# LemonATsu/UNet-PhaseGen

Measured on NVIDIA B200. Metric: audio_seconds_per_second_mag_to_phase_to_wave, higher is better.
Workload: dtype f16x3/f16x2/f16-fp32acc (two-product fp16 on d1,u2; single fp16 product = TF32 operand rounding on u1)

## Files before the change

unet-phasegen_b200/csrc/api.cu:

```cuda
#include <cstdarg>
#include <cstdio>

#include "common.cuh"
#include "conv_plan.h"

namespace pg {
static thread_local char g_err[512] = "";

void set_error(const char* fmt, ...) {
    va_list ap;
    va_start(ap, fmt);
    vsnprintf(g_err, sizeof(g_err), fmt, ap);
    va_end(ap);
}

int check_launch(const char* what) {
    cudaError_t e = cudaGetLastError();
    if (e != cudaSuccess) {
        set_error("%s: launch failed: %s", what, cudaGetErrorString(e));
        return PG_ERR_CUDA;
    }
    return PG_OK;
}
}

extern "C" const char* pg_last_error(void) { return pg::g_err; }
extern "C" int pg_abi_version(void) { return 4; }

extern "C" int pg_check_device(int* sm_count, int* cc_major, int* cc_minor) {
    int dev = 0, n = 0;
    if (cudaGetDeviceCount(&n) != cudaSuccess || n == 0) {
        cudaGetLastError();
        pg::set_error("no CUDA device: the phasegen path has no CPU fallback");
        return PG_ERR_CUDA;
    }
    cudaGetDevice(&dev);
    cudaDeviceProp p;
    if (cudaGetDeviceProperties(&p, dev) != cudaSuccess) { pg::set_error("cudaGetDeviceProperties failed"); return PG_ERR_CUDA; }
    if (sm_count) *sm_count = p.multiProcessorCount;
    if (cc_major) *cc_major = p.major;
    if (cc_minor) *cc_minor = p.minor;
    if (p.major != 10) {
        pg::set_error("device '%s' is sm_%d%d; this library is built for sm_100a (B200) only", p.name, p.major, p.minor);
        return PG_ERR_UNSUPPORTED;
    }
    return PG_OK;
}

extern "C" int pg_conv_stat_parts(const pg_conv_desc* d) {
    if (!d) return PG_ERR_INVALID;
    pg::ConvPlan pl;
    int rc = pg::conv_plan_build(d, &pl);
    if (rc != PG_OK) return rc;
    return pl.OS * pl.n_ntiles;
}

extern "C" int pg_conv_tc_plan(const pg_conv_desc* d, int* out, int n_out) {
    PG_REQUIRE(d && out && n_out >= 16, "pg_conv_tc_plan: need a descriptor and room for 16 ints");
    pg::ConvPlan p;
    int rc = pg::conv_plan_build(d, &p);
    if (rc != PG_OK) return rc;
    const int v[16] = {p.n_tile, p.n_ntiles, p.nb, p.strip_rows, p.pair, p.merged, p.mgroups, p.acc_stages,
                       p.n_chunks, p.n_cotiles, p.OS, p.IS, p.n_taps[0], p.n_taps[1], p.n_groups[0], p.n_groups[1]};
    for (int i = 0; i < 16; ++i) out[i] = v[i];
    if (n_out >= 17) out[16] = p.whole_clip;
    return PG_OK;
}
```

unet-phasegen_b200/csrc/conv_plan.h:

```cpp
#pragma once
#include <stdint.h>
#include <stdlib.h>

#include "../../include/phasegen.h"
#include "common.cuh"

namespace pg {

constexpr int kMaxTaps = 32;

struct ConvTap { int8_t w_idx; int8_t shift; int8_t parity; int8_t pad_; int32_t d; };
struct ConvGroup { int32_t row0; int8_t parity; int8_t n_taps; int8_t first_tap; int8_t pad_; };

struct ConvPlan {
    int B, C_in, C_out, L_in, L_out, k;
    int IS, OS;
    int n_tile, n_ntiles;
    int n_chunks, n_cotiles;
    int strip_rows;
    int nb;
    int acc_stages;
    int pair;
    int mgroups;
    int merged;
    int clip_group;
    int whole_clip;
    int out_rows, out_ld;
    int n_groups[2], n_taps[2];
    ConvGroup groups[2][kMaxTaps];
    ConvTap taps[2][kMaxTaps];
};

static inline int floordiv(int a, int b) { return (a >= 0) ? a / b : -((-a + b - 1) / b); }

static inline int conv_plan_build(const pg_conv_desc* d, ConvPlan* p) {
    const int s = d->stride, k = d->k, pad = d->pad;
    if (s < 1 || s > 2 || k < 1 || k > kMaxTaps) { set_error("conv plan: stride must be 1 or 2 and k <= %d (got s=%d k=%d)", kMaxTaps, s, k); return PG_ERR_UNSUPPORTED; }
    const bool tr = d->kind == PG_CONV_TRANSPOSE;
    const int L_expect = tr ? (d->L_in - 1) * s - 2 * pad + k : (d->L_in + 2 * pad - k) / s + 1;
    const bool len_ok = tr ? (d->L_out >= L_expect && d->L_out < L_expect + s) : d->L_out == L_expect;
    if (!len_ok || d->L_out < 1) { set_error("conv plan: L_out %d does not match geometry (expected %d)", d->L_out, L_expect); return PG_ERR_INVALID; }
    p->B = d->B; p->C_in = d->C_in; p->C_out = d->C_out; p->L_in = d->L_in; p->L_out = d->L_out; p->k = k;
    p->IS = tr ? 1 : s;
    p->OS = tr ? s : 1;
    p->out_rows = d->out_rows; p->out_ld = d->out_ld;
    p->n_chunks = d->C_in / 64; p->n_cotiles = d->C_out / 128;
    const int l_max = (d->L_out + p->OS - 1) / p->OS;
    p->n_ntiles = (l_max + 255) / 256;
    p->n_tile = (((l_max + p->n_ntiles - 1) / p->n_ntiles) + 15) / 16 * 16;
    int tpg = d->taps_per_group <= 0 ? 16 : d->taps_per_group;
    int max_shift = 0;
    for (int phi = 0; phi < 2; ++phi) { p->n_groups[phi] = 0; p->n_taps[phi] = 0; }
    for (int phi = 0; phi < p->OS; ++phi) {
        ConvTap t[kMaxTaps]; int n = 0;
        for (int kk = 0; kk < k; ++kk) {
            ConvTap e; e.w_idx = (int8_t)kk; e.shift = 0; e.pad_ = 0;
            if (tr) {
                int num = phi + pad - kk;
                if (((num % s) + s) % s != 0) continue;
                e.parity = 0; e.d = floordiv(num, s);
            } else {
                int off = kk - pad;
                int q = ((off % s) + s) % s;
                e.parity = (int8_t)q; e.d = (off - q) / s;
            }
            t[n++] = e;
        }
        for (int i = 1; i < n; ++i) {
            ConvTap e = t[i]; int j = i - 1;
            while (j >= 0 && (t[j].parity > e.parity || (t[j].parity == e.parity && t[j].d > e.d))) { t[j + 1] = t[j]; --j; }
            t[j + 1] = e;
        }
        int ng = 0, i = 0;
        while (i < n) {
            ConvGroup g; g.parity = t[i].parity; g.row0 = t[i].d; g.first_tap = (int8_t)i; g.pad_ = 0;
            int j = i;
            while (j < n && t[j].parity == g.parity && (j - i) < tpg && (t[j].d - g.row0) < tpg &&
                   (p->n_tile + (t[j].d - g.row0) <= 256)) {
                t[j].shift = (int8_t)(t[j].d - g.row0);
                if (t[j].shift > max_shift) max_shift = t[j].shift;
                ++j;
            }
            g.n_taps = (int8_t)(j - i);
            p->groups[phi][ng++] = g;
            i = j;
        }
        for (int q = 0; q < n; ++q) p->taps[phi][q] = t[q];
        p->n_groups[phi] = ng; p->n_taps[phi] = n;
    }
    p->pair = (d->tc_cta_pair != 1 && d->C_out % 256 == 0 && d->precision != PG_PREC_FP32_SIMT) ? 1 : 0;
    if (d->tc_cta_pair == 2 && !p->pair) { set_error("conv plan: CTA pairs need C_out %% 256 == 0 (got %d)", d->C_out); return PG_ERR_INVALID; }
    const int n_cta = p->pair ? p->n_tile / 2 : p->n_tile;
    p->strip_rows = (n_cta + max_shift + 7) / 8 * 8;
    if (p->strip_rows > 256) p->strip_rows = 256;
    p->nb = 1;
    const bool weight_bound = d->precision == PG_PREC_F16X2 || d->precision == PG_PREC_BF16 || d->precision == PG_PREC_F16;
    if ((p->n_ntiles == 1 || weight_bound) && d->max_clips_per_tile != 1) {
        const int planes = (d->precision == PG_PREC_BF16X3 || d->precision == PG_PREC_F16X3 || d->precision == PG_PREC_F16X2) ? 2 : 1;
        const int max_rows = (72 * 1024) / (planes * 128);
        int nb = 512 / p->n_tile;
        if (nb * p->strip_rows > max_rows) nb = max_rows / p->strip_rows;
        if (nb * p->n_tile <= 256 || (p->n_tile > 128 && !weight_bound)) {
            nb = 256 / p->n_tile;
            if (nb * p->strip_rows > 256) nb = 256 / p->strip_rows;
        }
        if (nb > 16) nb = 16;
        if (d->max_clips_per_tile > 1 && nb > d->max_clips_per_tile) nb = d->max_clips_per_tile;
        if (nb > d->B) nb = d->B;
        if (nb < 1) nb = 1;
        p->nb = nb;
    }
    if (const char* e = getenv("PG_TC_NB")) {
        int nb = atoi(e);
        if (nb >= 1 && nb * p->n_tile <= 512 && nb <= d->B) p->nb = nb;
    }
    p->merged = 0; p->mgroups = 1;
    {
        const int strip_full = (p->n_tile + max_shift + 7) / 8 * 8;
        const int step = p->pair ? 2 : 1;
        int nb_max = 256 / strip_full;
        if (nb_max > d->B) nb_max = d->B;
        if (d->max_clips_per_tile > 1 && nb_max > d->max_clips_per_tile) nb_max = d->max_clips_per_tile;
        nb_max -= nb_max % step;
        const char* off = getenv("PG_TC_MERGED");
        if (p->n_ntiles == 1 && nb_max >= 2 && d->max_clips_per_tile != 1 && !(off && atoi(off) == 0)) {
            const int units = (d->tc_max_ctas > 0 ? d->tc_max_ctas : 148) / (p->pair ? 2 : 1);
            const int slabs = (p->pair ? p->n_cotiles / 2 : p->n_cotiles) * p->OS;
            long best = -1; int best_nb = step;
            for (int nb = step; nb <= nb_max; nb += step) {
                const long tiles = (long)slabs * ((d->B + nb - 1) / nb);
                const long cost = ((tiles + units - 1) / units) * (64 + (long)nb * strip_full);
                if (best < 0 || cost <= best) { best = cost; best_nb = nb; }
            }
            p->merged = 1; p->nb = best_nb; p->strip_rows = strip_full;
            const char* g2 = getenv("PG_TC_MGROUPS");
            const int g_cap = g2 ? atoi(g2) : 2;
            const int planes_b = (d->precision == PG_PREC_BF16X3 || d->precision == PG_PREC_F16X3 || d->precision == PG_PREC_F16X2) ? 2 : 1;
            const char* fr = getenv("PG_TC_MG_FRAC");
            const double need = (fr ? atof(fr) : 0.8) * units;
            for (int g = 4; g >= 2 && weight_bound; --g) {
                if (g > g_cap || g * best_nb > d->B || g * best_nb * strip_full > 512) continue;
                const long tiles_g = (long)slabs * ((d->B + g * best_nb - 1) / (g * best_nb));
                const long slot_bytes = (long)planes_b * (g * best_nb / (p->pair ? 2 : 1)) * strip_full * 128;
                if ((double)tiles_g < need || 2 * slot_bytes > 120 * 1024) continue;
                p->mgroups = g; p->nb = g * best_nb;
                break;
            }
        }
    }
    p->whole_clip = 0;
    if (d->tc_whole_clip) {
        const int parts = p->OS * p->n_ntiles;
        if (p->merged && p->OS > 1) {
            set_error("conv plan: merged two-phase tiles do not hold a whole clip");
            return PG_ERR_UNSUPPORTED;
        }
        if (!p->merged) {
            if (parts * p->n_tile > 512) { set_error("conv plan: a whole clip needs %d accumulator columns (> 512)", parts * p->n_tile); return PG_ERR_UNSUPPORTED; }
            if (parts > 1) {
                p->whole_clip = 1;
                int nb = 1;
                if (weight_bound && 2 * parts * p->n_tile <= 512) nb = 2;
                if (nb > d->B) nb = d->B;
                const int planes = (d->precision == PG_PREC_BF16X3 || d->precision == PG_PREC_F16X3 || d->precision == PG_PREC_F16X2) ? 2 : 1;
                if (nb * p->n_ntiles * p->strip_rows * planes * 128 > 72 * 1024) nb = 1;
                if (p->n_ntiles * p->strip_rows * planes * 128 > 80 * 1024) {
                    set_error("conv plan: the %d strips of a whole clip (%d rows each) do not fit shared memory", p->n_ntiles, p->strip_rows);
                    return PG_ERR_UNSUPPORTED;
                }
                p->nb = nb;
            }
        }
    }
    {
        const int cols = p->merged ? p->nb * p->strip_rows : p->nb * p->n_tile * (p->whole_clip ? p->OS * p->n_ntiles : 1);
        if (cols > 512) { set_error("conv plan: tile needs %d accumulator columns (> 512)", cols); return PG_ERR_UNSUPPORTED; }
        p->acc_stages = cols <= 256 ? 2 : 1;
    }
    p->clip_group = d->B;
    return PG_OK;
}

}
```

unet-phasegen_b200/csrc/conv_tc.cu:

```cuda
#include "tc_ptx.cuh"
#include "conv_plan.h"

namespace pg {

struct ConvTcParams {
    ConvPlan plan;
    float* y;
    float4* stats;
    int n_a_slots;
    int b_slot_bytes;
    int n_terms;
    int f16;
    int base_offset_mode;
    int a_mn;
    int epi_mode;
    const float* gamma; const float* beta; float eps;
    ActDst dst0, dst1;
    float2* ss_out;
    const int* clip_rows;
};

constexpr int kThreads = 192;
constexpr int kATileBytes = 128 * 128;
constexpr int kMaxASlots = 8;

struct TileCoord { int co_tile, phase, b0, nt; };

__device__ __forceinline__ int n_bundles(const ConvPlan& p) { return (p.B + p.nb - 1) / p.nb; }
__device__ __forceinline__ int n_co_slabs(const ConvPlan& p) { return p.pair ? p.n_cotiles / 2 : p.n_cotiles; }
__device__ __forceinline__ int tile_OS(const ConvPlan& p) { return p.whole_clip ? 1 : p.OS; }
__device__ __forceinline__ int tile_NT(const ConvPlan& p) { return p.whole_clip ? 1 : p.n_ntiles; }
__device__ __forceinline__ int total_tiles(const ConvPlan& p) { return n_co_slabs(p) * tile_OS(p) * n_bundles(p) * tile_NT(p); }
__device__ __forceinline__ TileCoord decode_tile(const ConvPlan& p, int tile) {
    TileCoord c;
    const int OSx = tile_OS(p), NTx = tile_NT(p);
    const int nbg = n_bundles(p), G = p.clip_group, n_slabs = n_co_slabs(p) * OSx;
    const int tiles_full = n_slabs * G * NTx;
    const int g = tile / tiles_full, r = tile % tiles_full;
    int Gg = nbg - g * G; if (Gg > G) Gg = G;
    const int per_slab = Gg * NTx;
    const int slab = r / per_slab, r2 = r % per_slab;
    c.co_tile = slab / OSx; c.phase = slab % OSx;
    c.b0 = (g * G + r2 / NTx) * p.nb; c.nt = r2 % NTx;
    return c;
}

template <bool PAIR, bool RAGGED>
__global__ void __launch_bounds__(kThreads, 1)
conv_tc_kernel(const __grid_constant__ CUtensorMap map_w_hi, const __grid_constant__ CUtensorMap map_w_lo,
               const __grid_constant__ CUtensorMap map_x_hi, const __grid_constant__ CUtensorMap map_x_lo,
               const __grid_constant__ ConvTcParams prm) {
    extern __shared__ __align__(1024) uint8_t smem_raw[];
    const ConvPlan& pl = prm.plan;
    uint8_t* smem = reinterpret_cast<uint8_t*>((reinterpret_cast<uintptr_t>(smem_raw) + 1023) & ~uintptr_t(1023));
    const int nA = prm.n_a_slots;
    const int bPlane = prm.b_slot_bytes;
    const int a_planes = prm.n_terms == 3 ? 2 : 1;
    const int b_planes = prm.n_terms >= 2 ? 2 : 1;
    uint8_t* a_base = smem;
    uint8_t* b_base = a_base + (size_t)nA * a_planes * kATileBytes;
    uint64_t* bars = reinterpret_cast<uint64_t*>(b_base + 2 * (size_t)b_planes * bPlane);
    uint64_t* fullA = bars;
    uint64_t* emptyA = bars + kMaxASlots;
    uint64_t* fullB = bars + 2 * kMaxASlots;
    uint64_t* emptyB = fullB + 2;
    uint64_t* accFull = emptyB + 2;
    uint64_t* accEmpty = accFull + 2;
    uint32_t* tmem_slot = reinterpret_cast<uint32_t*>(accEmpty + 2);
    uint32_t* epi_tiles = reinterpret_cast<uint32_t*>(reinterpret_cast<uint8_t*>(bars) + 256);

    const int warp = __shfl_sync(0xffffffffu, (int)(threadIdx.x >> 5), 0), lane = threadIdx.x & 31;
    const int n_tiles = total_tiles(pl);
    const bool w_lo = prm.n_terms == 3, x_lo = prm.n_terms >= 2;

    if (warp == 0 && lane == 0) {
        tma_prefetch_desc(&map_w_hi); tma_prefetch_desc(&map_x_hi);
        if (w_lo) tma_prefetch_desc(&map_w_lo);
        if (x_lo) tma_prefetch_desc(&map_x_lo);
        for (int i = 0; i < nA; ++i) { mbar_init(fullA + i, 1); mbar_init(emptyA + i, 1); }
        for (int i = 0; i < 2; ++i) {
            mbar_init(fullB + i, 1); mbar_init(emptyB + i, 1);
            mbar_init(accFull + i, 1); mbar_init(accEmpty + i, PAIR ? 8 : 4);
        }
        fence_barrier_init();
    }
    if (warp == 1) { if (PAIR) tmem_alloc_pair(tmem_slot, 512); else tmem_alloc(tmem_slot, 512); }
    tc_fence_before();
    if (PAIR) cluster_sync_all(); else __syncthreads();
    tc_fence_after();
    const uint32_t tmem_base = __shfl_sync(0xffffffffu, *tmem_slot, 0);
    const int rank = PAIR ? (int)cluster_ctarank() : 0;
    const int tile0 = PAIR ? (int)(blockIdx.x >> 1) : (int)blockIdx.x;
    const int tile_step = PAIR ? (int)(gridDim.x >> 1) : (int)gridDim.x;
    const int half_n = pl.n_tile >> 1;
    const int nb_grp = pl.nb / pl.mgroups;
    const int nb_cta = (PAIR && pl.merged) ? nb_grp >> 1 : nb_grp;
    const int t_phases = pl.whole_clip ? pl.OS : 1;
    const int t_nts = pl.whole_clip ? pl.n_ntiles : 1;
    const int n_sub = pl.merged ? pl.mgroups : t_nts;

    if (warp == 0) {
        {
            uint32_t b_it = 0;
            int a_slot = 0; uint32_t a_ph = 0;
            const uint32_t grp_bytes = (uint32_t)nb_cta * pl.strip_rows * 128u;
            const uint32_t a_bytes = a_planes * kATileBytes;
            const uint32_t b_bytes = b_planes * (uint32_t)bPlane;
            for (int tile = tile0; tile < n_tiles; tile += tile_step) {
                TileCoord tc = decode_tile(pl, tile);
                if (PAIR) tc.co_tile = tc.co_tile * 2 + rank;
                const int m0 = tc.nt * pl.n_tile + ((PAIR && !pl.merged) ? rank * half_n : 0);
                const int clip0 = tc.b0 + ((PAIR && pl.merged) ? rank * nb_cta : 0);
                for (int ch = 0; ch < pl.n_chunks; ++ch) {
                  for (int ph = tc.phase; ph < tc.phase + t_phases; ++ph) {
                    const int ng = pl.n_groups[ph];
                    for (int g = 0; g < ng; ++g) {
                        const ConvGroup grp = pl.groups[ph][g];
                        {
                            const int s = b_it & 1; const uint32_t bph = (b_it >> 1) & 1;
                            mbar_wait(emptyB + s, bph ^ 1);
                            uint8_t* dst = b_base + (size_t)s * b_planes * bPlane;
                            if (elect_one()) {
                                if (PAIR) { if (rank == 0) mbar_expect_tx(fullB + s, 2 * b_bytes); }
                                else mbar_expect_tx(fullB + s, b_bytes);
                                for (int sub = 0; sub < n_sub; ++sub) {
                                    uint8_t* dg = dst + (size_t)sub * grp_bytes;
                                    const int cg = clip0 + (pl.merged ? sub * nb_grp : 0);
                                    const int r0 = m0 + (pl.merged ? 0 : sub * pl.n_tile) + grp.row0;
                                    if (PAIR) {
                                        tma_load_4d_pair(dg, &map_x_hi, fullB + s, ch * 64, grp.parity, r0, cg);
                                        if (x_lo) tma_load_4d_pair(dg + bPlane, &map_x_lo, fullB + s, ch * 64, grp.parity, r0, cg);
                                    } else {
                                        tma_load_4d(dg, &map_x_hi, fullB + s, ch * 64, grp.parity, r0, cg);
                                        if (x_lo) tma_load_4d(dg + bPlane, &map_x_lo, fullB + s, ch * 64, grp.parity, r0, cg);
                                    }
                                }
                            }
                            __syncwarp();
                            ++b_it;
                        }
                        for (int j = 0; j < grp.n_taps; ++j) {
                            const int w_idx = pl.taps[ph][grp.first_tap + j].w_idx;
                            const int s = a_slot; const uint32_t aph = a_ph;
                            mbar_wait(emptyA + s, aph ^ 1);
                            uint8_t* dst = a_base + (size_t)s * a_planes * kATileBytes;
                            if (elect_one()) {
                                if (!PAIR) mbar_expect_tx(fullA + s, a_bytes);
                                else if (rank == 0) mbar_expect_tx(fullA + s, 2 * a_bytes);
                                auto load_w = [&](uint8_t* d, const CUtensorMap* m, int c0, int c1) {
                                    if (PAIR) tma_load_3d_pair(d, m, fullA + s, c0, c1, w_idx);
                                    else tma_load_3d(d, m, fullA + s, c0, c1, w_idx);
                                };
                                if (prm.a_mn) {
                                    for (int h = 0; h < 2; ++h) {
                                        load_w(dst + h * 8192, &map_w_hi, tc.co_tile * 128 + h * 64, ch * 64);
                                        if (w_lo) load_w(dst + kATileBytes + h * 8192, &map_w_lo, tc.co_tile * 128 + h * 64, ch * 64);
                                    }
                                } else {
                                    load_w(dst, &map_w_hi, ch * 64, tc.co_tile * 128);
                                    if (w_lo) load_w(dst + kATileBytes, &map_w_lo, ch * 64, tc.co_tile * 128);
                                }
                            }
                            __syncwarp();
                            if (++a_slot == nA) { a_slot = 0; a_ph ^= 1; }
                        }
                    }
                  }
                }
            }
        }
    } else if (warp == 1) {
        if (rank == 0) {
            uint32_t b_it = 0, t_it = 0;
            int a_slot = 0; uint32_t a_ph = 0;
            const int n_mma = pl.merged ? nb_grp * pl.strip_rows : pl.n_tile;
            const int n_outer = pl.merged ? 1 : t_nts, n_inner = pl.merged ? pl.mgroups : pl.nb;
            const uint32_t dcol_step = pl.merged ? (uint32_t)n_mma : (uint32_t)(pl.n_tile * t_phases * t_nts);
            const uint32_t idesc = (make_idesc_bf16(n_mma, PAIR ? 256 : 128) & ~(prm.f16 ? ((7u << 7) | (7u << 10)) : 0u)) |
                                   (prm.a_mn ? (1u << 15) : 0u);
            const bool a_mn = prm.a_mn != 0;
            auto mma = [&](uint32_t d, uint32_t da, uint32_t db, uint32_t acc_flag) {
                if (elect_one()) { if (PAIR) umma_words_pair(d, da, db, idesc, acc_flag); else umma_words(d, da, db, idesc, acc_flag); }
            };
            const uint32_t a_step = a_mn ? (2048u >> 4) : (32u >> 4);
            auto commit = [&](uint64_t* bar) {
                if (elect_one()) { if (PAIR) umma_commit_pair(bar); else umma_commit(bar); }
                __syncwarp();
            };
            for (int tile = tile0; tile < n_tiles; tile += tile_step, ++t_it) {
                TileCoord tc = decode_tile(pl, tile);
                const int acc = pl.acc_stages == 2 ? (t_it & 1) : 0;
                const uint32_t acc_ph = pl.acc_stages == 2 ? ((t_it >> 1) & 1) : (t_it & 1);
                mbar_wait_sleep(accEmpty + acc, acc_ph ^ 1, 200);
                tc_fence_after();
                const uint32_t d_tmem = tmem_base + acc * 256;
                const uint32_t strip_bytes = (uint32_t)pl.strip_rows * 128u;
                const uint32_t clip_step = (pl.merged ? (uint32_t)nb_cta * strip_bytes : strip_bytes) >> 4;
                for (int ch = 0; ch < pl.n_chunks; ++ch) {
                  for (int ph = tc.phase; ph < tc.phase + t_phases; ++ph) {
                    const int ng = pl.n_groups[ph];
                    const uint32_t dcol_ph = d_tmem + (uint32_t)((ph - tc.phase) * t_nts * pl.n_tile);
                    for (int g = 0; g < ng; ++g) {
                        const ConvGroup grp = pl.groups[ph][g];
                        const int bs = b_it & 1; const uint32_t bph = (b_it >> 1) & 1;
                        mbar_wait(fullB + bs, bph);
                        tc_fence_after();
                        const uint32_t b_hi = smem_u32(b_base + (size_t)bs * b_planes * bPlane);
                        const uint32_t b_lo = b_hi + bPlane;
                        for (int j = 0; j < grp.n_taps; ++j) {
                            const ConvTap tp = pl.taps[ph][grp.first_tap + j];
                            const int as = a_slot; const uint32_t aph = a_ph;
                            mbar_wait(fullA + as, aph);
                            tc_fence_after();
                            const uint32_t a_hi = smem_u32(a_base + (size_t)as * a_planes * kATileBytes);
                            const uint32_t a_lo = a_hi + kATileBytes;
                            const uint32_t sh = (uint32_t)tp.shift * 128u;
                            const uint32_t acc_first = (ch | g | j) ? 1u : 0u;
                            const uint32_t aw_hi = a_mn ? desc_lo_sw128_mn(a_hi, 8192) : desc_lo_sw128(a_hi);
                            const uint32_t aw_lo = a_mn ? desc_lo_sw128_mn(a_lo, 8192) : desc_lo_sw128(a_lo);
                            uint32_t bw_hi = desc_lo_sw128(b_hi + sh), bw_lo = desc_lo_sw128(b_lo + sh);
                            for (int o = 0; o < n_outer; ++o) {
                                uint32_t dcol = dcol_ph + (uint32_t)o * (uint32_t)pl.n_tile;
                                for (int c = 0; c < n_inner; ++c, bw_hi += clip_step, bw_lo += clip_step, dcol += dcol_step) {
                                    if (w_lo) {
#pragma unroll
                                        for (uint32_t kk = 0; kk < 4; ++kk) {
                                            mma(dcol, aw_lo + kk * a_step, bw_hi + kk * 2, kk == 0 ? acc_first : 1u);
                                            mma(dcol, aw_hi + kk * a_step, bw_lo + kk * 2, 1);
                                            mma(dcol, aw_hi + kk * a_step, bw_hi + kk * 2, 1);
                                        }
                                    } else if (x_lo) {
#pragma unroll
                                        for (uint32_t kk = 0; kk < 4; ++kk) {
                                            mma(dcol, aw_hi + kk * a_step, bw_lo + kk * 2, kk == 0 ? acc_first : 1u);
                                            mma(dcol, aw_hi + kk * a_step, bw_hi + kk * 2, 1);
                                        }
                                    } else {
#pragma unroll
                                        for (uint32_t kk = 0; kk < 4; ++kk) mma(dcol, aw_hi + kk * a_step, bw_hi + kk * 2, kk == 0 ? acc_first : 1u);
                                    }
                                }
                            }
                            commit(emptyA + as);
                            if (++a_slot == nA) { a_slot = 0; a_ph ^= 1; }
                        }
                        commit(emptyB + bs);
                        ++b_it;
                    }
                  }
                }
                commit(accFull + acc);
            }
        }
    } else {
        const int q = warp & 3;
        uint32_t* tile = epi_tiles + q * 512;
        uint32_t t_it = 0;
        const int n_parts = t_phases * t_nts;
        const int col_pitch = pl.merged ? pl.strip_rows : pl.n_tile * n_parts;
        bool bad_range = false;
        auto store_f32 = [&](float* base, size_t off0, size_t row_pitch, const float* v, int nv) {
#pragma unroll
            for (int i = 0; i < 16; ++i) tile[i * 32 + lane] = __float_as_uint(v[i]);
            __syncwarp();
#pragma unroll
            for (int t = 0; t < 4; ++t) {
                const int idx = lane + 32 * t, r = idx >> 3, part = idx & 7;
                if (r < nv) {
                    const uint4 w = *reinterpret_cast<const uint4*>(tile + r * 32 + part * 4);
                    *reinterpret_cast<uint4*>(base + off0 + (size_t)r * row_pitch + part * 4) = w;
                }
            }
            __syncwarp();
        };
        auto store_split = [&](const ActDst& d, size_t off0, size_t row_pitch, const float* v, int nv) {
            const int fmt = fmt_of_dtype(d.dtype);
#pragma unroll
            for (int i = 0; i < 16; ++i) {
                const float a = leaky(v[i], d.slope);
                uint16_t h, l;
                split16(a, fmt, h, l);
                if (fmt == PG_FMT_F16 && i < nv) bad_range |= !f16_fits(a);
                tile[i * 32 + lane] = (uint32_t)h | ((uint32_t)l << 16);
            }
            __syncwarp();
            const bool two = d.dtype == PG_DT_BF16_SPLIT || d.dtype == PG_DT_F16_SPLIT;
#pragma unroll
            for (int t = 0; t < 2; ++t) {
                const int idx = lane + 32 * t, r = idx >> 2, part = idx & 3;
                if (r < nv) {
                    const uint4 w0 = *reinterpret_cast<const uint4*>(tile + r * 32 + part * 8);
                    const uint4 w1 = *reinterpret_cast<const uint4*>(tile + r * 32 + part * 8 + 4);
                    uint4 hv, lv;
                    hv.x = __byte_perm(w0.x, w0.y, 0x5410); hv.y = __byte_perm(w0.z, w0.w, 0x5410);
                    hv.z = __byte_perm(w1.x, w1.y, 0x5410); hv.w = __byte_perm(w1.z, w1.w, 0x5410);
                    lv.x = __byte_perm(w0.x, w0.y, 0x7632); lv.y = __byte_perm(w0.z, w0.w, 0x7632);
                    lv.z = __byte_perm(w1.x, w1.y, 0x7632); lv.w = __byte_perm(w1.z, w1.w, 0x7632);
                    const size_t o = off0 + (size_t)r * row_pitch + part * 8;
                    *reinterpret_cast<uint4*>(static_cast<uint16_t*>(d.hi) + o) = hv;
                    if (two) *reinterpret_cast<uint4*>(static_cast<uint16_t*>(d.lo) + o) = lv;
                }
            }
            __syncwarp();
        };
        for (int tile_i = tile0; tile_i < n_tiles; tile_i += tile_step, ++t_it) {
            TileCoord tc = decode_tile(pl, tile_i);
            if (PAIR) tc.co_tile = tc.co_tile * 2 + rank;
            const int acc = pl.acc_stages == 2 ? (t_it & 1) : 0;
            const uint32_t acc_ph = pl.acc_stages == 2 ? ((t_it >> 1) & 1) : (t_it & 1);
            mbar_wait_sleep(accFull + acc, acc_ph, 1000);
            tc_fence_after();
            const int co_base = tc.co_tile * 128 + q * 32;
            const int co = co_base + lane;
            auto part_geom = [&](int p, int L, int& phase, int& m0, int& n_valid) {
                phase = tc.phase + p / t_nts;
                m0 = (tc.nt + p % t_nts) * pl.n_tile;
                const int l_phase = (L - phase + pl.OS - 1) / pl.OS;
                n_valid = l_phase - m0; if (n_valid > pl.n_tile) n_valid = pl.n_tile; if (n_valid < 0) n_valid = 0;
            };
            for (int c = 0; c < pl.nb; ++c) {
                const int b = tc.b0 + c;
                if (b >= pl.B) break;
                const int L_b = RAGGED ? min(__ldg(prm.clip_rows + b), pl.L_out) : pl.L_out;
                const uint32_t tclip = tmem_base + acc * 256 + c * col_pitch + ((uint32_t)(q * 32) << 16);
                if (prm.epi_mode == PG_EPI_RAW) {
                    for (int p = 0; p < n_parts; ++p) {
                        int phase, m0, n_valid;
                        part_geom(p, L_b, phase, m0, n_valid);
                        const uint32_t taddr = tclip + p * pl.n_tile;
                        float sum = 0.f;
                        for (int c0 = 0; c0 < n_valid; c0 += 16) {
                            float v[16];
                            tmem_ld16(taddr + c0, v);
#pragma unroll
                            for (int i = 0; i < 16; ++i) if (c0 + i < n_valid) sum += v[i];
                        }
                        const float mean = n_valid > 0 ? sum / (float)n_valid : 0.f;
                        float m2 = 0.f;
                        const size_t row_pitch = (size_t)pl.OS * pl.out_ld;
                        for (int c0 = 0; c0 < n_valid; c0 += 16) {
                            float v[16];
                            tmem_ld16(taddr + c0, v);
#pragma unroll
                            for (int i = 0; i < 16; ++i) if (c0 + i < n_valid) { const float d = v[i] - mean; m2 += d * d; }
                            const size_t off0 = ((size_t)b * pl.out_rows + (size_t)(m0 + c0) * pl.OS + phase) * pl.out_ld + co_base;
                            store_f32(prm.y, off0, row_pitch, v, n_valid - c0);
                        }
                        if (prm.stats) {
                            const int P = pl.OS * pl.n_ntiles;
                            const int pi = phase * pl.n_ntiles + m0 / pl.n_tile;
                            prm.stats[((size_t)b * P + pi) * pl.C_out + co] = make_float4((float)n_valid, mean, m2, 0.f);
                        }
                    }
                } else {
                    float sc = 1.f, sh = 0.f;
                    if (prm.epi_mode == PG_EPI_NORM_ACT) {
                        float sum = 0.f; int n_tot = 0;
                        for (int p = 0; p < n_parts; ++p) {
                            int phase, m0, n_valid;
                            part_geom(p, L_b, phase, m0, n_valid);
                            n_tot += n_valid;
                            for (int c0 = 0; c0 < n_valid; c0 += 16) {
                                float v[16];
                                tmem_ld16(tclip + p * pl.n_tile + c0, v);
#pragma unroll
                                for (int i = 0; i < 16; ++i) if (c0 + i < n_valid) sum += v[i];
                            }
                        }
                        const float mean = n_tot > 0 ? sum / (float)n_tot : 0.f;
                        float m2 = 0.f;
                        for (int p = 0; p < n_parts; ++p) {
                            int phase, m0, n_valid;
                            part_geom(p, L_b, phase, m0, n_valid);
                            for (int c0 = 0; c0 < n_valid; c0 += 16) {
                                float v[16];
                                tmem_ld16(tclip + p * pl.n_tile + c0, v);
#pragma unroll
                                for (int i = 0; i < 16; ++i) if (c0 + i < n_valid) { const float d = v[i] - mean; m2 += d * d; }
                            }
                        }
                        const float var = n_tot > 0 ? m2 / (float)n_tot : 0.f;
                        sc = (prm.gamma ? __ldg(prm.gamma + co) : 1.f) * rsqrtf(var + prm.eps);
                        sh = (prm.beta ? __ldg(prm.beta + co) : 0.f) - mean * sc;
                        if (prm.ss_out) prm.ss_out[(size_t)b * pl.C_out + co] = make_float2(sc, sh);
                    }
                    for (int p = 0; p < n_parts; ++p) {
                        int phase, m0, n_valid, n_own = 0;
                        part_geom(p, pl.L_out, phase, m0, n_valid);
                        if (RAGGED) { int ph_, m0_; part_geom(p, L_b, ph_, m0_, n_own); }
                        for (int c0 = 0; c0 < n_valid; c0 += 16) {
                            float v[16];
                            tmem_ld16(tclip + p * pl.n_tile + c0, v);
#pragma unroll
                            for (int i = 0; i < 16; ++i) v[i] = fmaf(v[i], sc, sh);
                            if (RAGGED) {
#pragma unroll
                                for (int i = 0; i < 16; ++i) if (c0 + i >= n_own) v[i] = 0.f;
                            }
                            const size_t row0 = (size_t)(m0 + c0) * pl.OS + phase;
#pragma unroll
                            for (int k = 0; k < 2; ++k) {
                                const ActDst& d = k ? prm.dst1 : prm.dst0;
                                if (!d.dtype) continue;
                                const size_t off0 = (size_t)b * d.batch_stride + row0 * d.ld + d.ch_off + co_base;
                                if (d.dtype == PG_DT_F32) {
                                    float a[16];
#pragma unroll
                                    for (int i = 0; i < 16; ++i) a[i] = leaky(v[i], d.slope);
                                    store_f32(static_cast<float*>(d.hi), off0, (size_t)pl.OS * d.ld, a, n_valid - c0);
                                } else {
                                    store_split(d, off0, (size_t)pl.OS * d.ld, v, n_valid - c0);
                                }
                            }
                        }
                    }
                }
            }
            tc_fence_before();
            __syncwarp();
            if (lane == 0) { if (PAIR) mbar_arrive_leader(accEmpty + acc); else mbar_arrive(accEmpty + acc); }
        }
        if (bad_range) {
            if (prm.dst0.range_flag) atomicOr(prm.dst0.range_flag, 1);
            else if (prm.dst1.range_flag) atomicOr(prm.dst1.range_flag, 1);
        }
    }
    tc_fence_before();
    if (PAIR) cluster_sync_all(); else __syncthreads();
    if (warp == 1) { tc_fence_after(); if (PAIR) tmem_dealloc_pair(tmem_base, 512); else tmem_dealloc(tmem_base, 512); }
}

static EncodeTiledFn get_encode() {
    static EncodeTiledFn fn = nullptr;
    if (!fn) {
        void* p = nullptr;
        cudaDriverEntryPointQueryResult qres;
        if (cudaGetDriverEntryPoint("cuTensorMapEncodeTiled", &p, cudaEnableDefault, &qres) == cudaSuccess &&
            qres == cudaDriverEntryPointSuccess)
            fn = reinterpret_cast<EncodeTiledFn>(p);
    }
    return fn;
}

int encode_bf16_map(CUtensorMap* map, const void* base, int rank, const uint64_t* dims, const uint64_t* strides_bytes,
                       const uint32_t* box, const char* what) {
    EncodeTiledFn enc = get_encode();
    if (!enc) { set_error("cuTensorMapEncodeTiled entry point not available"); return PG_ERR_CUDA; }
    cuuint64_t d[5], s[5]; cuuint32_t bx[5], es[5];
    for (int i = 0; i < rank; ++i) { d[i] = dims[i]; bx[i] = box[i]; es[i] = 1; }
    for (int i = 0; i + 1 < rank; ++i) s[i] = strides_bytes[i];
    CUresult r = enc(map, CU_TENSOR_MAP_DATA_TYPE_BFLOAT16, rank, const_cast<void*>(base), d, s, bx, es,
                     CU_TENSOR_MAP_INTERLEAVE_NONE, CU_TENSOR_MAP_SWIZZLE_128B, CU_TENSOR_MAP_L2_PROMOTION_L2_256B,
                     CU_TENSOR_MAP_FLOAT_OOB_FILL_NONE);
    if (r != CUDA_SUCCESS) { set_error("cuTensorMapEncodeTiled(%s) failed with CUresult %d", what, (int)r); return PG_ERR_CUDA; }
    return PG_OK;
}

void device_limits(int* sm_count, int* max_smem) {
    static int sm_dev[kMaxDevices] = {}, smem_dev[kMaxDevices] = {};
    const int slot = current_device_slot();
    if (!sm_dev[slot]) {
        int dev = 0; cudaGetDevice(&dev);
        cudaDeviceGetAttribute(&sm_dev[slot], cudaDevAttrMultiProcessorCount, dev);
        cudaDeviceGetAttribute(&smem_dev[slot], cudaDevAttrMaxSharedMemoryPerBlockOptin, dev);
    }
    *sm_count = sm_dev[slot]; *max_smem = smem_dev[slot];
}

}

extern "C" int pg_conv_epilogue_supported(const pg_conv_desc* d, int mode) {
    using namespace pg;
    PG_REQUIRE(d, "pg_conv_epilogue_supported: null descriptor");
    if (mode == PG_EPI_RAW) return 1;
    if (mode != PG_EPI_ACT && mode != PG_EPI_NORM_ACT) return 0;
    if (d->precision == PG_PREC_FP32_SIMT || d->C_in % 64 || d->C_out % 128) return 0;
    if (mode == PG_EPI_ACT) return 1;
    pg_conv_desc dd = *d;
    dd.tc_whole_clip = 1;
    ConvPlan pl;
    if (conv_plan_build(&dd, &pl) != PG_OK) return 0;
    return (pl.whole_clip || (pl.OS == 1 && pl.n_ntiles == 1)) ? 1 : 0;
}

static int conv_tc_launch(const pg_conv_desc* d, const uint16_t* x_hi, const uint16_t* x_lo, const uint16_t* w_hi,
                          const uint16_t* w_lo, float* y, float* stats, const pg_conv_epilogue* epi, const int* out_rows,
                          pg_stream stream) {
    using namespace pg;
    const int epi_mode = epi ? epi->mode : PG_EPI_RAW;
    PG_REQUIRE(d && x_hi && w_hi && (y || epi_mode != PG_EPI_RAW), "pg_conv_tc: null pointer");
    PG_REQUIRE(epi_mode == PG_EPI_RAW || epi_mode == PG_EPI_ACT || epi_mode == PG_EPI_NORM_ACT, "pg_conv_tc: bad epilogue mode %d", epi_mode);
    PG_REQUIRE(d->precision >= PG_PREC_BF16X3 && d->precision <= PG_PREC_F16, "pg_conv_tc: precision must be BF16X3, BF16, F16X3, F16X2 or F16");
    const int n_terms = (d->precision == PG_PREC_BF16X3 || d->precision == PG_PREC_F16X3) ? 3 : d->precision == PG_PREC_F16X2 ? 2 : 1;
    const bool three = n_terms == 3;
    PG_REQUIRE(n_terms < 3 || w_lo, "pg_conv_tc: weight lo plane required for the three-product precisions");
    PG_REQUIRE(n_terms < 2 || x_lo, "pg_conv_tc: activation lo plane required for this precision");
    PG_REQUIRE(d->C_in % 64 == 0 && d->C_out % 128 == 0, "pg_conv_tc: needs C_in %% 64 == 0 and C_out %% 128 == 0 (got %d, %d)", d->C_in, d->C_out);
    PG_REQUIRE(d->in_ld % 8 == 0, "pg_conv_tc: input row pitch must be a multiple of 8 elements");
    PG_REQUIRE(d->tc_base_offset_mode == 0, "pg_conv_tc: descriptor base-offset mode 0 is the only supported one (the UMMA swizzle is a "
               "function of the absolute shared-memory address: profiles/r01_tc_probe.log)");
    ConvTcParams prm;
    pg_conv_desc d_local = *d;
    if (const char* e = getenv("PG_TC_PAIR")) d_local.tc_cta_pair = atoi(e);
    d_local.tc_whole_clip = epi_mode == PG_EPI_NORM_ACT ? 1 : 0;
    d = &d_local;
    int rc = conv_plan_build(d, &prm.plan);
    if (rc != PG_OK) return rc;
    const ConvPlan& pl = prm.plan;
    prm.epi_mode = epi_mode; prm.gamma = nullptr; prm.beta = nullptr; prm.eps = 1e-5f; prm.ss_out = nullptr;
    prm.clip_rows = out_rows;
    const bool ragged = out_rows != nullptr;
    if ((rc = to_act_dst(nullptr, 0, &prm.dst0, "pg_conv_tc", "dst0")) != PG_OK) return rc;
    prm.dst1 = prm.dst0;
    if (epi_mode != PG_EPI_RAW) {
        PG_REQUIRE(epi_mode != PG_EPI_NORM_ACT || pl.whole_clip || (pl.OS == 1 && pl.n_ntiles == 1),
                   "pg_conv_tc: the fused per-clip norm needs a whole clip per tile (L_out %d does not fit 512 accumulator columns)", pl.L_out);
        if ((rc = to_act_dst(&epi->dst0, d->C_out, &prm.dst0, "pg_conv_tc", "dst0")) != PG_OK) return rc;
        if ((rc = to_act_dst(&epi->dst1, d->C_out, &prm.dst1, "pg_conv_tc", "dst1")) != PG_OK) return rc;
        PG_REQUIRE(prm.dst0.dtype || prm.dst1.dtype, "pg_conv_tc: fused epilogue without a destination");
        for (const ActDst* a : {&prm.dst0, &prm.dst1})
            PG_REQUIRE(!a->dtype || (a->ld % 8 == 0 && a->ch_off % 8 == 0 && a->batch_stride % 8 == 0 && (reinterpret_cast<uintptr_t>(a->hi) & 15) == 0 &&
                                      (reinterpret_cast<uintptr_t>(a->lo) & 15) == 0),
                       "pg_conv_tc: fused-epilogue destinations need 16-byte aligned planes and ld, ch_off, batch_stride multiples of 8");
        prm.gamma = epi->gamma; prm.beta = epi->beta; prm.eps = epi->eps; prm.ss_out = reinterpret_cast<float2*>(epi->scale_shift);
    } else {
        PG_REQUIRE(d->out_ld % 4 == 0 && (reinterpret_cast<uintptr_t>(y) & 15) == 0, "pg_conv_tc: y must be 16-byte aligned with out_ld a multiple of 4");
    }
    int g_sm_count, g_max_smem;
    device_limits(&g_sm_count, &g_max_smem);
    prm.y = y; prm.stats = reinterpret_cast<float4*>(stats);
    prm.n_terms = n_terms;
    prm.f16 = (d->precision == PG_PREC_F16X3 || d->precision == PG_PREC_F16X2 || d->precision == PG_PREC_F16) ? 1 : 0;
    prm.base_offset_mode = d->tc_base_offset_mode;
    prm.a_mn = d->weights_mn_major ? 1 : 0;
    const int nb_grp = pl.nb / pl.mgroups;
    const int nb_cta = (pl.pair && pl.merged) ? nb_grp / 2 : nb_grp;
    prm.b_slot_bytes = (pl.merged ? pl.mgroups : (pl.whole_clip ? pl.n_ntiles : 1)) * nb_cta * pl.strip_rows * 128;
    const int a_planes = n_terms == 3 ? 2 : 1, b_planes = n_terms >= 2 ? 2 : 1;
    const int fixed = 2 * b_planes * prm.b_slot_bytes + 1024  + 256  + 8192  +
                      (pl.merged ? 2048 : 0);
    int nA = (g_max_smem - fixed) / (a_planes * kATileBytes);
    if (nA > kMaxASlots) nA = kMaxASlots;
    PG_REQUIRE(nA >= 2, "pg_conv_tc: strip of %d rows leaves no room for the weight ring", pl.strip_rows);
    prm.n_a_slots = nA;
    const size_t smem_bytes = (size_t)fixed + (size_t)nA * a_planes * kATileBytes;

    CUtensorMap mw_hi, mw_lo, mx_hi, mx_lo;
    {
        const uint64_t inner = prm.a_mn ? d->C_out : d->C_in, outer = prm.a_mn ? d->C_in : d->C_out;
        uint64_t dims[3] = {inner, outer, (uint64_t)d->k};
        uint64_t str[2] = {inner * 2, inner * outer * 2};
        uint32_t box[3] = {64, prm.a_mn ? 64u : 128u, 1};
        if ((rc = encode_bf16_map(&mw_hi, w_hi, 3, dims, str, box, "w_hi")) != PG_OK) return rc;
        if ((rc = encode_bf16_map(&mw_lo, three ? w_lo : w_hi, 3, dims, str, box, "w_lo")) != PG_OK) return rc;
    }
    {
        const int IS = pl.IS;
        uint64_t dims[4] = {(uint64_t)d->C_in, (uint64_t)IS, (uint64_t)((d->L_in + IS - 1) / IS), (uint64_t)d->B};
        uint64_t str[3] = {(uint64_t)d->in_ld * 2, (uint64_t)d->in_ld * 2 * IS, (uint64_t)d->in_rows * d->in_ld * 2};
        uint32_t box[4] = {64, 1, (uint32_t)pl.strip_rows, (uint32_t)nb_cta};
        PG_REQUIRE(d->in_rows >= ((d->L_in + IS - 1) / IS) * IS, "pg_conv_tc: in_rows %d too small for L_in %d at stride %d", d->in_rows, d->L_in, IS);
        if ((rc = encode_bf16_map(&mx_hi, x_hi, 4, dims, str, box, "x_hi")) != PG_OK) return rc;
        if ((rc = encode_bf16_map(&mx_lo, n_terms >= 2 ? x_lo : x_hi, 4, dims, str, box, "x_lo")) != PG_OK) return rc;
    }
    const bool pair = pl.pair != 0;
    auto kernel = pair ? (ragged ? conv_tc_kernel<true, true> : conv_tc_kernel<true, false>)
                       : (ragged ? conv_tc_kernel<false, true> : conv_tc_kernel<false, false>);
    {
        static size_t configured_dev[kMaxDevices][4] = {};
        const int variant = 2 * pair + ragged;
        size_t* configured = configured_dev[current_device_slot()];
        if (smem_bytes > configured[variant]) {
            cudaError_t e = cudaFuncSetAttribute(kernel, cudaFuncAttributeMaxDynamicSharedMemorySize, (int)smem_bytes);
            if (e != cudaSuccess) { set_error("conv_tc: cannot opt in to %zu bytes of shared memory: %s", smem_bytes, cudaGetErrorString(e)); return PG_ERR_CUDA; }
            configured[variant] = smem_bytes;
        }
    }
    {
        const int nbg = (pl.B + pl.nb - 1) / pl.nb;
        const double bundle_bytes = (double)pl.nb * d->in_rows * d->in_ld * (n_terms >= 2 ? 4.0 : 2.0);
        int G = (int)(64.0e6 / bundle_bytes);
        if (const char* e = getenv("PG_TC_CLIP_GROUP")) G = atoi(e);
        if (G < 1) G = 1;
        if (G > nbg) G = nbg;
        prm.plan.clip_group = G;
    }
    const int n_tiles = (pair ? pl.n_cotiles / 2 : pl.n_cotiles) * ((pl.B + pl.nb - 1) / pl.nb) * (pl.whole_clip ? 1 : pl.OS * pl.n_ntiles);
    int units = pair ? g_sm_count / 2 : g_sm_count;
    if (const char* e = getenv("PG_TC_MAX_CTAS")) {
        const int cap = atoi(e);
        if (cap > 0 && units > (pair ? cap / 2 : cap)) units = pair ? cap / 2 : cap;
    }
    if (d->tc_max_ctas > 0 && units > (pair ? (d->tc_max_ctas + 1) / 2 : d->tc_max_ctas)) units = pair ? (d->tc_max_ctas + 1) / 2 : d->tc_max_ctas;
    if (units > n_tiles) units = n_tiles;
    cudaLaunchConfig_t cfg = {};
    cfg.gridDim = dim3(pair ? 2 * units : units);
    cfg.blockDim = dim3(kThreads);
    cfg.dynamicSmemBytes = smem_bytes;
    cfg.stream = reinterpret_cast<cudaStream_t>(stream);
    cudaLaunchAttribute attr[1];
    attr[0].id = cudaLaunchAttributeClusterDimension;
    attr[0].val.clusterDim.x = pair ? 2 : 1; attr[0].val.clusterDim.y = 1; attr[0].val.clusterDim.z = 1;
    cfg.attrs = attr; cfg.numAttrs = 1;
    cudaError_t le = cudaLaunchKernelEx(&cfg, kernel, mw_hi, mw_lo, mx_hi, mx_lo, prm);
    if (le != cudaSuccess) { set_error("conv_tc_kernel launch failed: %s", cudaGetErrorString(le)); return PG_ERR_CUDA; }
    return check_launch("conv_tc_kernel");
}

extern "C" int pg_conv_tc(const pg_conv_desc* d, const uint16_t* x_hi, const uint16_t* x_lo, const uint16_t* w_hi,
                          const uint16_t* w_lo, float* y, float* stats, const pg_conv_epilogue* epi, pg_stream stream) {
    return conv_tc_launch(d, x_hi, x_lo, w_hi, w_lo, y, stats, epi, nullptr, stream);
}

extern "C" int pg_conv_tc_ragged(const pg_conv_desc* d, const uint16_t* x_hi, const uint16_t* x_lo, const uint16_t* w_hi,
                                 const uint16_t* w_lo, float* y, float* stats, const pg_conv_epilogue* epi, const int* out_rows,
                                 pg_stream stream) {
    PG_REQUIRE(out_rows, "pg_conv_tc_ragged: null per-clip row table");
    return conv_tc_launch(d, x_hi, x_lo, w_hi, w_lo, y, stats, epi, out_rows, stream);
}
```

unet-phasegen_b200/csrc/tc_ptx.cuh:

```cuda
#pragma once
#include <cuda.h>

#include <cstdio>
#include <cstdlib>

#include "common.cuh"

namespace pg {

__device__ __forceinline__ uint32_t smem_u32(const void* p) { return (uint32_t)__cvta_generic_to_shared(p); }

__device__ __forceinline__ void mbar_init(uint64_t* bar, uint32_t count) {
    asm volatile("mbarrier.init.shared::cta.b64 [%0], %1;" ::"r"(smem_u32(bar)), "r"(count));
}
__device__ __forceinline__ void mbar_expect_tx(uint64_t* bar, uint32_t bytes) {
    asm volatile("mbarrier.arrive.expect_tx.shared::cta.b64 _, [%0], %1;" ::"r"(smem_u32(bar)), "r"(bytes) : "memory");
}
__device__ __forceinline__ void mbar_arrive(uint64_t* bar) {
    asm volatile("mbarrier.arrive.shared::cta.b64 _, [%0];" ::"r"(smem_u32(bar)) : "memory");
}
__device__ __forceinline__ bool mbar_try_wait(uint64_t* bar, uint32_t parity) {
    uint32_t ok;
    asm volatile(
        "{\n\t.reg .pred p;\n\t"
        "mbarrier.try_wait.parity.shared::cta.b64 p, [%1], %2;\n\t"
        "selp.u32 %0, 1, 0, p;\n\t}"
        : "=r"(ok) : "r"(smem_u32(bar)), "r"(parity) : "memory");
    return ok != 0;
}
__device__ __forceinline__ void mbar_wait(uint64_t* bar, uint32_t parity) {
    if (mbar_try_wait(bar, parity)) return;
    const long long t0 = clock64();
    for (uint32_t spins = 1; !mbar_try_wait(bar, parity); ++spins) {
        if ((spins & 1023u) == 0 && clock64() - t0 > 4000000000ll) {
            printf("phasegen conv_tc: mbarrier timeout (block %d thread %d bar %u parity %u)\n",
                   (int)blockIdx.x, (int)threadIdx.x, smem_u32(bar), parity);
            __trap();
        }
    }
}
__device__ __forceinline__ void mbar_wait_sleep(uint64_t* bar, uint32_t parity, unsigned ns) {
    if (mbar_try_wait(bar, parity)) return;
    const long long t0 = clock64();
    for (uint32_t spins = 1; !mbar_try_wait(bar, parity); ++spins) {
        __nanosleep(ns);
        if ((spins & 255u) == 0 && clock64() - t0 > 4000000000ll) {
            printf("phasegen conv_tc: mbarrier timeout (block %d thread %d bar %u parity %u)\n",
                   (int)blockIdx.x, (int)threadIdx.x, smem_u32(bar), parity);
            __trap();
        }
    }
}
__device__ __forceinline__ bool elect_one() {
    uint32_t pred;
    asm volatile("{\n\t.reg .pred p;\n\telect.sync _|p, 0xffffffff;\n\tselp.u32 %0, 1, 0, p;\n\t}" : "=r"(pred));
    return pred != 0;
}
__device__ __forceinline__ void fence_barrier_init() { asm volatile("fence.mbarrier_init.release.cluster;" ::: "memory"); }
__device__ __forceinline__ void fence_proxy_async() { asm volatile("fence.proxy.async.shared::cta;" ::: "memory"); }
__device__ __forceinline__ void tc_fence_before() { asm volatile("tcgen05.fence::before_thread_sync;" ::: "memory"); }
__device__ __forceinline__ void tc_fence_after() { asm volatile("tcgen05.fence::after_thread_sync;" ::: "memory"); }

__device__ __forceinline__ void tma_load_3d(void* dst, const CUtensorMap* map, uint64_t* bar, int c0, int c1, int c2) {
    asm volatile(
        "cp.async.bulk.tensor.3d.shared::cluster.global.tile.mbarrier::complete_tx::bytes [%0], [%1, {%3, %4, %5}], [%2];"
        ::"r"(smem_u32(dst)), "l"(map), "r"(smem_u32(bar)), "r"(c0), "r"(c1), "r"(c2) : "memory");
}
__device__ __forceinline__ void tma_load_4d(void* dst, const CUtensorMap* map, uint64_t* bar, int c0, int c1, int c2, int c3) {
    asm volatile(
        "cp.async.bulk.tensor.4d.shared::cluster.global.tile.mbarrier::complete_tx::bytes [%0], [%1, {%3, %4, %5, %6}], [%2];"
        ::"r"(smem_u32(dst)), "l"(map), "r"(smem_u32(bar)), "r"(c0), "r"(c1), "r"(c2), "r"(c3) : "memory");
}
__device__ __forceinline__ void tma_prefetch_desc(const CUtensorMap* map) {
    asm volatile("prefetch.tensormap [%0];" ::"l"(map) : "memory");
}

__device__ __forceinline__ void tmem_alloc(uint32_t* dst_smem, uint32_t cols) {
    asm volatile("tcgen05.alloc.cta_group::1.sync.aligned.shared::cta.b32 [%0], %1;" ::"r"(smem_u32(dst_smem)), "r"(cols) : "memory");
    asm volatile("tcgen05.relinquish_alloc_permit.cta_group::1.sync.aligned;" ::: "memory");
}
__device__ __forceinline__ void tmem_dealloc(uint32_t addr, uint32_t cols) {
    asm volatile("tcgen05.dealloc.cta_group::1.sync.aligned.b32 %0, %1;" ::"r"(addr), "r"(cols) : "memory");
}
__device__ __forceinline__ void umma_bf16(uint32_t d_tmem, uint64_t a_desc, uint64_t b_desc, uint32_t idesc, uint32_t accumulate) {
    asm volatile(
        "{\n\t.reg .pred p;\n\t"
        "setp.ne.b32 p, %4, 0;\n\t"
        "tcgen05.mma.cta_group::1.kind::f16 [%0], %1, %2, %3, p;\n\t}"
        ::"r"(d_tmem), "l"(a_desc), "l"(b_desc), "r"(idesc), "r"(accumulate) : "memory");
}
__device__ __forceinline__ void umma_commit(uint64_t* bar) {
    asm volatile("tcgen05.commit.cta_group::1.mbarrier::arrive::one.shared::cluster.b64 [%0];" ::"r"(smem_u32(bar)) : "memory");
}
__device__ __forceinline__ void tmem_ld16(uint32_t taddr, float* v) {
    uint32_t r[16];
    asm volatile(
        "tcgen05.ld.sync.aligned.32x32b.x16.b32 {%0,%1,%2,%3,%4,%5,%6,%7,%8,%9,%10,%11,%12,%13,%14,%15}, [%16];"
        : "=r"(r[0]), "=r"(r[1]), "=r"(r[2]), "=r"(r[3]), "=r"(r[4]), "=r"(r[5]), "=r"(r[6]), "=r"(r[7]),
          "=r"(r[8]), "=r"(r[9]), "=r"(r[10]), "=r"(r[11]), "=r"(r[12]), "=r"(r[13]), "=r"(r[14]), "=r"(r[15])
        : "r"(taddr));
    asm volatile("tcgen05.wait::ld.sync.aligned;" ::: "memory");
#pragma unroll
    for (int i = 0; i < 16; ++i) v[i] = __uint_as_float(r[i]);
}

constexpr uint32_t kPeerBitMask = 0xFEFFFFFFu;

__device__ __forceinline__ uint32_t cluster_ctarank() { uint32_t r; asm volatile("mov.u32 %0, %%cluster_ctarank;" : "=r"(r)); return r; }
__device__ __forceinline__ void cluster_sync_all() {
    asm volatile("barrier.cluster.arrive.release.aligned;" ::: "memory");
    asm volatile("barrier.cluster.wait.acquire.aligned;" ::: "memory");
}
__device__ __forceinline__ void tma_load_3d_pair(void* dst, const CUtensorMap* map, uint64_t* bar, int c0, int c1, int c2) {
    asm volatile(
        "cp.async.bulk.tensor.3d.cta_group::2.shared::cluster.global.mbarrier::complete_tx::bytes [%0], [%1, {%3, %4, %5}], [%2];"
        ::"r"(smem_u32(dst)), "l"(map), "r"(smem_u32(bar) & kPeerBitMask), "r"(c0), "r"(c1), "r"(c2) : "memory");
}
__device__ __forceinline__ void tma_load_4d_pair(void* dst, const CUtensorMap* map, uint64_t* bar, int c0, int c1, int c2, int c3) {
    asm volatile(
        "cp.async.bulk.tensor.4d.cta_group::2.shared::cluster.global.mbarrier::complete_tx::bytes [%0], [%1, {%3, %4, %5, %6}], [%2];"
        ::"r"(smem_u32(dst)), "l"(map), "r"(smem_u32(bar) & kPeerBitMask), "r"(c0), "r"(c1), "r"(c2), "r"(c3) : "memory");
}
__device__ __forceinline__ void tmem_alloc_pair(uint32_t* dst_smem, uint32_t cols) {
    asm volatile("tcgen05.alloc.cta_group::2.sync.aligned.shared::cta.b32 [%0], %1;" ::"r"(smem_u32(dst_smem)), "r"(cols) : "memory");
    asm volatile("tcgen05.relinquish_alloc_permit.cta_group::2.sync.aligned;" ::: "memory");
}
__device__ __forceinline__ void tmem_dealloc_pair(uint32_t addr, uint32_t cols) {
    asm volatile("tcgen05.dealloc.cta_group::2.sync.aligned.b32 %0, %1;" ::"r"(addr), "r"(cols) : "memory");
}
__device__ __forceinline__ void umma_bf16_pair(uint32_t d_tmem, uint64_t a_desc, uint64_t b_desc, uint32_t idesc, uint32_t accumulate) {
    asm volatile(
        "{\n\t.reg .pred p;\n\t"
        "setp.ne.b32 p, %4, 0;\n\t"
        "tcgen05.mma.cta_group::2.kind::f16 [%0], %1, %2, %3, p;\n\t}"
        ::"r"(d_tmem), "l"(a_desc), "l"(b_desc), "r"(idesc), "r"(accumulate) : "memory");
}
__device__ __forceinline__ void umma_commit_pair(uint64_t* bar) {
    asm volatile("tcgen05.commit.cta_group::2.mbarrier::arrive::one.shared::cluster.multicast::cluster.b64 [%0], %1;"
                 ::"r"(smem_u32(bar)), "h"((uint16_t)3) : "memory");
}
__device__ __forceinline__ void mbar_arrive_leader(uint64_t* bar) {
    asm volatile("mbarrier.arrive.release.cluster.shared::cluster.b64 _, [%0];" ::"r"(smem_u32(bar) & kPeerBitMask) : "memory");
}

__device__ __forceinline__ uint64_t make_desc_sw128(uint32_t saddr, int base_offset_mode) {
    uint64_t d = 0;
    d |= (uint64_t)((saddr & 0x3FFFF) >> 4);
    d |= (uint64_t)0 << 16;
    d |= (uint64_t)(1024 >> 4) << 32;
    d |= (uint64_t)1 << 46;
    if (base_offset_mode) d |= (uint64_t)((saddr >> 7) & 7) << 49;
    d |= (uint64_t)2 << 61;
    return d;
}
constexpr uint32_t kDescHiSw128 = (1024u >> 4) | (1u << 14) | (2u << 29);
__device__ __forceinline__ uint32_t desc_lo_sw128(uint32_t saddr) { return (saddr & 0x3FFFF) >> 4; }
__device__ __forceinline__ uint32_t desc_lo_sw128_mn(uint32_t saddr, uint32_t lbo_bytes) {
    return ((saddr & 0x3FFFF) >> 4) | (((lbo_bytes >> 4) & 0x3FFF) << 16);
}
__device__ __forceinline__ void umma_words(uint32_t d_tmem, uint32_t a_lo, uint32_t b_lo, uint32_t idesc, uint32_t accumulate) {
    asm volatile(
        "{\n\t.reg .pred p;\n\t.reg .b64 da, db;\n\t"
        "setp.ne.b32 p, %4, 0;\n\t"
        "mov.b64 da, {%1, %5};\n\t"
        "mov.b64 db, {%2, %5};\n\t"
        "tcgen05.mma.cta_group::1.kind::f16 [%0], da, db, %3, p;\n\t}"
        ::"r"(d_tmem), "r"(a_lo), "r"(b_lo), "r"(idesc), "r"(accumulate), "r"(kDescHiSw128) : "memory");
}
__device__ __forceinline__ void umma_words_pair(uint32_t d_tmem, uint32_t a_lo, uint32_t b_lo, uint32_t idesc, uint32_t accumulate) {
    asm volatile(
        "{\n\t.reg .pred p;\n\t.reg .b64 da, db;\n\t"
        "setp.ne.b32 p, %4, 0;\n\t"
        "mov.b64 da, {%1, %5};\n\t"
        "mov.b64 db, {%2, %5};\n\t"
        "tcgen05.mma.cta_group::2.kind::f16 [%0], da, db, %3, p;\n\t}"
        ::"r"(d_tmem), "r"(a_lo), "r"(b_lo), "r"(idesc), "r"(accumulate), "r"(kDescHiSw128) : "memory");
}

__device__ __forceinline__ uint32_t make_idesc_bf16(int n, int m = 128) {
    return (1u << 4) | (1u << 7) | (1u << 10) | ((uint32_t)(n >> 3) << 17) | ((uint32_t)(m >> 4) << 24);
}


__device__ __forceinline__ uint64_t make_desc_sw128_mn(uint32_t saddr, uint32_t lbo_bytes) {
    uint64_t d = 0;
    d |= (uint64_t)((saddr & 0x3FFFF) >> 4);
    d |= (uint64_t)((lbo_bytes >> 4) & 0x3FFF) << 16;
    d |= (uint64_t)(1024 >> 4) << 32;
    d |= (uint64_t)1 << 46;
    d |= (uint64_t)2 << 61;
    return d;
}
__device__ __forceinline__ uint32_t make_idesc_bf16_mn(int n) {
    return make_idesc_bf16(n) | (1u << 15) | (1u << 16);
}

typedef CUresult (*EncodeTiledFn)(CUtensorMap*, CUtensorMapDataType, cuuint32_t, void*, const cuuint64_t*,
                                  const cuuint64_t*, const cuuint32_t*, const cuuint32_t*, CUtensorMapInterleave,
                                  CUtensorMapSwizzle, CUtensorMapL2promotion, CUtensorMapFloatOOBfill);

int encode_bf16_map(CUtensorMap* map, const void* base, int rank, const uint64_t* dims, const uint64_t* strides_bytes,
                    const uint32_t* box, const char* what);
void device_limits(int* sm_count, int* max_smem);

}
```

unet-phasegen_b200/phasegen/ops.py:

```python
import ctypes as C
import math

import torch

from . import _lib
from ._lib import (ActDst, ConvDesc, ConvEpilogue, PG_EPI_ACT, PG_EPI_NORM_ACT, PG_EPI_RAW, PG_CONV, PG_CONV_TRANSPOSE, PG_DT_BF16, PG_DT_BF16_SPLIT, PG_DT_F16,
                   PG_DT_F16_SPLIT, PG_DT_F32, PG_DT_NONE, PG_FMT_BF16, PG_FMT_F16, PG_PREC_BF16, PG_PREC_BF16X3,
                   PG_PREC_F16X2, PG_PREC_F16X3, PG_PREC_FP32_SIMT, PG_SPEC_CARTESIAN, PG_SPEC_POLAR_LOG,
                   PG_SPEC_POLAR_MAG, PG_STFT_LOGMAG, PG_STFT_REIM)

SUPPORTED_N_FFT = (256, 512, 1024, 2048)


def _stream(t=None):
    dev = t.device if isinstance(t, torch.Tensor) and t.is_cuda else None
    return C.c_void_p(torch.cuda.current_stream(dev).cuda_stream)


def _ptr(t):
    return C.c_void_p(t.data_ptr()) if t is not None else C.c_void_p(0)


def _fmt(t):
    if t is None or t.dtype == torch.bfloat16:
        return PG_FMT_BF16
    if t.dtype == torch.float16:
        return PG_FMT_F16
    raise RuntimeError(f"phasegen: operand planes must be bfloat16 or float16, got {t.dtype}")


def _need_cuda(t, name, dtype=torch.float32):
    if not isinstance(t, torch.Tensor) or not t.is_cuda:
        raise RuntimeError(f"phasegen: `{name}` must be a CUDA tensor (there is no CPU path)")
    if t.dtype != dtype:
        raise RuntimeError(f"phasegen: `{name}` must be {dtype}, got {t.dtype}")
    if t.device.index != torch.cuda.current_device():
        raise RuntimeError(f"phasegen: `{name}` lives on {t.device} but the current device is cuda:{torch.cuda.current_device()}; "
                           "wrap the call in `with torch.cuda.device(tensor.device):`")
    _lib.require_device(t.device.index)
    return t.contiguous()


_twiddles = {}


def twiddle(n_fft, device):
    key = (n_fft, str(device))
    if key not in _twiddles:
        m = torch.arange(n_fft, dtype=torch.float64)
        ang = -2.0 * math.pi * m / n_fft
        _twiddles[key] = torch.stack([torch.cos(ang), torch.sin(ang)], 1).float().contiguous().to(device)
    return _twiddles[key]


def check_stft_geometry(n_fft, hop):
    if n_fft not in SUPPORTED_N_FFT or hop * 4 != n_fft:
        raise RuntimeError(f"phasegen: n_fft must be one of {SUPPORTED_N_FFT} with hop = n_fft/4 "
                           f"(got n_fft={n_fft}, hop={hop})")


def _lengths(t, B, name):
    t = _need_cuda(t, name, torch.int32)
    if t.numel() != B:
        raise RuntimeError(f"phasegen: `{name}` must hold one entry per clip ({B}), got {t.numel()}")
    return t


def stft(wave, n_fft, hop, mode=PG_STFT_LOGMAG, want_second=True, operand=None, clip_samples=None, clip_frames=None):
    check_stft_geometry(n_fft, hop)
    wave = _need_cuda(wave, "wave")
    if wave.dim() != 2:
        raise RuntimeError("phasegen.stft: wave must be [B, N]")
    B, N = wave.shape
    T = 1 + N // hop
    Cb = n_fft // 2
    a = torch.empty(B, T, Cb, device=wave.device, dtype=torch.float32)
    b = torch.empty_like(a) if want_second else None
    hi, lo, bs = operand if operand is not None else (None, None, 0)
    if clip_samples is not None or clip_frames is not None:
        _lib.call("pg_stft_ragged", _ptr(wave), B, N, n_fft, hop, _ptr(twiddle(n_fft, wave.device)), mode,
                  _ptr(a), _ptr(b), _ptr(hi), _ptr(lo), bs, _fmt(hi), _ptr(_lengths(clip_samples, B, "clip_samples")),
                  _ptr(_lengths(clip_frames, B, "clip_frames")), _stream())
        return a, b
    _lib.call("pg_stft", _ptr(wave), B, N, n_fft, hop, _ptr(twiddle(n_fft, wave.device)), mode,
              _ptr(a), _ptr(b), _ptr(hi), _ptr(lo), bs, _fmt(hi), _stream())
    return a, b


def stft_project(wave, mag, n_fft, hop, out=None):
    check_stft_geometry(n_fft, hop)
    wave = _need_cuda(wave, "wave")
    mag = _need_cuda(mag, "mag")
    B, N = wave.shape
    T = 1 + N // hop
    if tuple(mag.shape) != (B, T, n_fft // 2):
        raise RuntimeError(f"phasegen.stft_project: mag must be [{B}, {T}, {n_fft // 2}], got {tuple(mag.shape)}")
    re, im = out if out is not None else (torch.empty_like(mag), torch.empty_like(mag))
    _lib.call("pg_stft_project", _ptr(wave), B, N, n_fft, hop, _ptr(twiddle(n_fft, wave.device)), _ptr(mag),
              _ptr(re), _ptr(im), _stream())
    return re, im


def stft_pairs(wave, n_fft, hop, mean=0.0, std=1.0):
    check_stft_geometry(n_fft, hop)
    wave = _need_cuda(wave, "wave")
    B, N = wave.shape
    T = 1 + N // hop
    lm = torch.empty(B, T, n_fft // 2, device=wave.device, dtype=torch.float32)
    ph = torch.empty_like(lm)
    _lib.call("pg_stft_pairs", _ptr(wave), B, N, n_fft, hop, _ptr(twiddle(n_fft, wave.device)), float(mean), float(std),
              _ptr(lm), _ptr(ph), _stream())
    return lm, ph


def istft(a, b, mode, n_fft, hop, normalize=True, check_finite=True, out=None, b_scale_shift=None, bad_out=None,
          clip_frames=None, clip_samples=None):
    check_stft_geometry(n_fft, hop)
    a = _need_cuda(a, "a")
    b = _need_cuda(b, "b") if b is not None else None
    B, T, Cb = a.shape
    if Cb != n_fft // 2 or (b is not None and b.shape != a.shape):
        raise RuntimeError("phasegen.istft: inputs must be [B, T, n_fft/2] and of equal shape")
    n = (T - 1) * hop
    if out is not None and (tuple(out.shape) != (B, n) or out.dtype != torch.float32 or not out.is_cuda or not out.is_contiguous()):
        raise RuntimeError(f"phasegen.istft: `out` must be a contiguous CUDA float32 [{B}, {n}] tensor")
    wave = out if out is not None else torch.empty(B, n, device=a.device, dtype=torch.float32)
    peak = torch.empty(B, device=a.device, dtype=torch.float32)
    bad = bad_out if bad_out is not None else torch.empty(B, device=a.device, dtype=torch.int32)
    per_clip = 0
    if b_scale_shift is not None:
        b_scale_shift = _need_cuda(b_scale_shift, "b_scale_shift")
        if b_scale_shift.numel() not in (2 * Cb, 2 * Cb * B):
            raise RuntimeError("phasegen.istft: b_scale_shift must hold (scale, shift) per bin, for all clips or per clip")
        per_clip = int(b_scale_shift.numel() == 2 * Cb * B and B > 1)
    if clip_frames is not None or clip_samples is not None:
        _lib.call("pg_istft_ragged", _ptr(a), _ptr(b), mode, B, T, n_fft, hop, _ptr(twiddle(n_fft, a.device)),
                  _ptr(wave), _ptr(peak), _ptr(bad), _ptr(b_scale_shift), per_clip,
                  _ptr(_lengths(clip_frames, B, "clip_frames")), _ptr(_lengths(clip_samples, B, "clip_samples")), _stream())
    else:
        _lib.call("pg_istft", _ptr(a), _ptr(b), mode, B, T, n_fft, hop, _ptr(twiddle(n_fft, a.device)),
                  _ptr(wave), _ptr(peak), _ptr(bad), _ptr(b_scale_shift), per_clip, _stream())
    if normalize:
        _lib.call("pg_peak_normalize", _ptr(wave), _ptr(peak), B, n, _stream())
    if check_finite and bool(bad.any().item()):
        raise ValueError("Audio buffer is not finite everywhere")
    return wave, peak


def transpose(src, dst=None, dst_hi=None, dst_lo=None, dst_batch_stride=None, dst_ld=None, range_flag=None):
    src = _need_cuda(src, "src")
    B, R, S = src.shape
    if dst is None and dst_hi is None:
        dst = torch.empty(B, S, R, device=src.device, dtype=torch.float32)
    ld = R if dst_ld is None else dst_ld
    bs = S * ld if dst_batch_stride is None else dst_batch_stride
    _lib.call("pg_transpose", _ptr(src), B, R, S, R * S, _ptr(dst), _ptr(dst_hi), _ptr(dst_lo), bs, ld, _fmt(dst_hi), _ptr(range_flag), _stream())
    return dst


def conv_desc(kind, B, C_in, C_out, L_in, k, stride, pad, in_rows, in_ld, precision, L_out=None,
              out_rows=None, out_ld=None, taps_per_group=0, base_offset_mode=0, max_ctas=0, max_clips_per_tile=0, weights_mn_major=0, cta_pair=0,
              whole_clip=0):
    if L_out is None:
        L_out = (L_in - 1) * stride - 2 * pad + k if kind == PG_CONV_TRANSPOSE else (L_in + 2 * pad - k) // stride + 1
    return ConvDesc(kind, B, C_in, C_out, L_in, L_out, k, stride, pad, in_rows, in_ld,
                    L_out if out_rows is None else out_rows, C_out if out_ld is None else out_ld,
                    precision, taps_per_group, base_offset_mode, max_ctas, max_clips_per_tile, weights_mn_major, cta_pair, whole_clip)


def pack_weight(w, kind, want_tc=True, want_simt=False, plane_dtype=torch.bfloat16, want_lo=True):
    w = _need_cuda(w.detach(), "weight")
    if kind == PG_CONV_TRANSPOSE:
        C_in, C_out, k = w.shape
    else:
        C_out, C_in, k = w.shape
    hi = lo = simt = None
    if want_tc:
        hi = torch.empty(k, C_out, C_in, device=w.device, dtype=plane_dtype)
        lo = torch.empty_like(hi) if want_lo else None
    if want_simt:
        simt = torch.empty(k, C_in, C_out, device=w.device, dtype=torch.float32)
    _lib.call("pg_pack_weight", _ptr(w), kind, C_in, C_out, k, _ptr(hi), _ptr(lo), _ptr(simt), _fmt(hi), _stream())
    return hi, lo, simt


def conv_tc(desc, x_hi, x_lo, w_hi, w_lo, y, stats, epilogue=None, out_rows=None):
    if out_rows is not None:
        _lib.call("pg_conv_tc_ragged", C.byref(desc), _ptr(x_hi), _ptr(x_lo), _ptr(w_hi), _ptr(w_lo), _ptr(y), _ptr(stats),
                  C.byref(epilogue) if epilogue is not None else None, _ptr(_lengths(out_rows, desc.B, "out_rows")), _stream())
        return
    _lib.call("pg_conv_tc", C.byref(desc), _ptr(x_hi), _ptr(x_lo), _ptr(w_hi), _ptr(w_lo), _ptr(y), _ptr(stats),
              C.byref(epilogue) if epilogue is not None else None, _stream())


_NO_DST = ActDst(None, None, 0, 0, 0, PG_DT_NONE, 1.0, None)


def conv_epilogue(mode, dst0, dst1=None, gamma=None, beta=None, eps=1e-5, scale_shift=None):
    return ConvEpilogue(mode, gamma.data_ptr() if gamma is not None else None, beta.data_ptr() if beta is not None else None,
                        float(eps), dst0, dst1 if dst1 is not None else _NO_DST,
                        scale_shift.data_ptr() if scale_shift is not None else None)


def conv_epilogue_supported(desc, mode):
    r = _lib.load().pg_conv_epilogue_supported(C.byref(desc), mode)
    if r < 0:
        raise RuntimeError(f"pg_conv_epilogue_supported failed ({r}): {_lib.last_error()}")
    return bool(r)


def conv_stat_parts(desc):
    p = _lib.load().pg_conv_stat_parts(C.byref(desc))
    if p <= 0:
        raise RuntimeError(f"pg_conv_stat_parts failed ({p}): {_lib.last_error()}")
    return p


_PLAN_KEYS = ("n_tile", "n_ntiles", "nb", "strip_rows", "pair", "merged", "mgroups", "acc_stages", "n_chunks", "n_cotiles",
              "OS", "IS", "taps0", "taps1", "groups0", "groups1", "whole_clip")


def conv_plan(desc, whole_clip=None):
    d = ConvDesc.from_buffer_copy(desc)
    if whole_clip is not None:
        d.tc_whole_clip = int(whole_clip)
    out = (C.c_int * 17)()
    if _lib.load().pg_conv_tc_plan(C.byref(d), out, 17) != 0:
        return None
    pl = dict(zip(_PLAN_KEYS, out))
    slabs = pl["n_cotiles"] // 2 if pl["pair"] else pl["n_cotiles"]
    parts = 1 if pl["whole_clip"] else pl["OS"] * pl["n_ntiles"]
    pl["tiles"] = slabs * parts * -(-d.B // pl["nb"])
    pl["units"] = 74 if pl["pair"] else 148
    return pl


def conv_simt(desc, x, w_simt, y):
    _lib.call("pg_conv_simt", C.byref(desc), _ptr(x), _ptr(w_simt), _ptr(y), _stream())


def channel_stats(y, B, L, Cn, rows, ld, stats):
    _lib.call("pg_channel_stats", _ptr(y), B, L, Cn, rows, ld, _ptr(stats), _stream())


def bn_finalize(stats, B, P, Cn, per_clip, gamma, beta, eps, scale_shift, mean_var=None):
    _lib.call("pg_bn_finalize", _ptr(stats), B, P, Cn, int(per_clip), _ptr(gamma), _ptr(beta), eps,
              _ptr(scale_shift), _ptr(mean_var), _stream())


def act_dst(hi, lo, batch_stride, ld, ch_off, dtype, slope, range_flag=None):
    return ActDst(hi.data_ptr() if hi is not None else None, lo.data_ptr() if lo is not None else None,
                  batch_stride, ld, ch_off, dtype, slope, range_flag.data_ptr() if range_flag is not None else None)


def bn_running_update(mean_var, running_mean, running_var, momentum, unbias):
    Cn = running_mean.numel()
    for t, name in ((mean_var, "mean_var"), (running_mean, "running_mean"), (running_var, "running_var")):
        _need_cuda(t, name)
        if t.dtype != torch.float32 or not t.is_contiguous():
            raise RuntimeError(f"phasegen.bn_running_update: {name} must be a contiguous float32 CUDA tensor")
    if mean_var.numel() < 2 * Cn or running_var.numel() != Cn:
        raise RuntimeError("phasegen.bn_running_update: shapes do not match")
    _lib.call("pg_bn_running_update", _ptr(mean_var), _ptr(running_mean), _ptr(running_var), Cn, float(momentum), float(unbias), _stream())


def bn_from_running(running_mean, running_var, gamma, beta, eps, scale_shift, mean_var=None):
    G, Cn = scale_shift.shape[0], scale_shift.shape[1]
    _lib.call("pg_bn_from_running", _ptr(running_mean), _ptr(running_var), _ptr(gamma), _ptr(beta), float(eps), Cn, G,
              _ptr(scale_shift), _ptr(mean_var), _stream())


def bn_act(y, B, L, Cn, rows, ld, scale_shift, per_clip, dst0, dst1=None, clip_rows=None):
    if clip_rows is not None:
        _lib.call("pg_bn_act_ragged", _ptr(y), B, L, Cn, rows, ld, _ptr(scale_shift), int(per_clip),
                  C.byref(dst0), C.byref(dst1) if dst1 is not None else None, _ptr(_lengths(clip_rows, B, "clip_rows")), _stream())
        return
    _lib.call("pg_bn_act", _ptr(y), B, L, Cn, rows, ld, _ptr(scale_shift), int(per_clip),
              C.byref(dst0), C.byref(dst1) if dst1 is not None else None, _stream())


def grad_src(g, ld, ch_off, slope):
    return _lib.GradSrc(g.data_ptr(), ld, ch_off, slope)


def phase_loss(out_cl, logmag_cl, phase_cl, d_out, partial, loss3, mag_weight=0.2):
    B, T, C2 = out_cl.shape
    _lib.call("pg_phase_loss", _ptr(out_cl), _ptr(logmag_cl), _ptr(phase_cl), B * T, C2 // 2, mag_weight,
              _ptr(d_out), _ptr(partial), partial.shape[0], _ptr(loss3), _stream(), n_kernels=2)


def bn_bwd(z, B, L, Cn, scale_shift, mean_var, eps, g0, g1, partial, coef, dgamma, dbeta, dz_hi, dz_lo, dz_rows, dz_dtype):
    n_chunks = partial.shape[0] if partial is not None else 0
    _lib.call("pg_bn_bwd", _ptr(z), B, L, Cn, _ptr(scale_shift), _ptr(mean_var), eps, C.byref(g0),
              C.byref(g1) if g1 is not None else None, _ptr(partial), n_chunks, _ptr(coef), _ptr(dgamma), _ptr(dbeta),
              _ptr(dz_hi), _ptr(dz_lo), dz_rows, dz_dtype, _stream(), n_kernels=3 if scale_shift is not None else 1)


def wgrad_tc(desc, x_hi, x_lo, g_hi, g_lo, g_rows, dw_packed):
    dt = PG_DT_BF16 if dw_packed.dtype == torch.bfloat16 else PG_DT_F32
    _lib.call("pg_wgrad_tc", C.byref(desc), _ptr(x_hi), _ptr(x_lo), _ptr(g_hi), _ptr(g_lo), g_rows, _ptr(dw_packed), dt, _stream())


def wgrad_simt(desc, x, g, g_rows, dw_packed):
    _lib.call("pg_wgrad_simt", C.byref(desc), _ptr(x), _ptr(g), g_rows, _ptr(dw_packed), _stream())


def unpack_grad(packed, kind, out):
    k, C_out, C_in = packed.shape
    _lib.call("pg_unpack_grad", _ptr(packed), kind, C_in, C_out, k, _ptr(out), _stream())


def adam_step(p, g, m, v, lr, beta1, beta2, eps, step, grad_scale=1.0, w_hi=None, w_lo=None):
    gdt = PG_DT_BF16 if g.dtype == torch.bfloat16 else PG_DT_F32
    _lib.call("pg_adam_step", _ptr(p), _ptr(g), gdt, _ptr(m), _ptr(v), p.numel(), lr, beta1, beta2, eps, step, grad_scale,
              _ptr(w_hi), _ptr(w_lo), _stream())


def cast_split(src, hi, lo=None, range_flag=None):
    _lib.call("pg_cast_split", _ptr(src), src.numel(), _ptr(hi), _ptr(lo), _fmt(hi), _ptr(range_flag), _stream())


def packed_view(weight, kind):
    w = weight.detach()
    v = w.permute(2, 1, 0) if kind == PG_CONV_TRANSPOSE else w.permute(2, 0, 1)
    return v if v.is_contiguous() else None


def to_packed_storage(weight, kind):
    w = weight.detach()
    packed = (w.permute(2, 1, 0) if kind == PG_CONV_TRANSPOSE else w.permute(2, 0, 1)).contiguous()
    return packed.permute(2, 1, 0) if kind == PG_CONV_TRANSPOSE else packed.permute(1, 2, 0)
```

unet-phasegen_b200/phasegen/unet.py:

```python
import torch

from . import ops
from ._lib import (PG_CONV, PG_CONV_TRANSPOSE, PG_DT_BF16, PG_DT_BF16_SPLIT, PG_DT_F16, PG_DT_F16_SPLIT, PG_DT_F32, PG_EPI_ACT,
                   PG_EPI_NORM_ACT, PG_EPI_RAW, PG_PREC_BF16, PG_PREC_BF16X3, PG_PREC_F16, PG_PREC_F16X2, PG_PREC_F16X3,
                   PG_PREC_FP32_SIMT, PRECISIONS)

BN_EPS_DEFAULT = 1e-5
DEFAULT_TAPS_PER_GROUP = 16
F16MIX_FAST_LAYERS = ("d1", "u1", "u2")
F16MIX1_SINGLE_LAYERS = ("u1",)
_SPLIT_PRECS = (PG_PREC_BF16X3, PG_PREC_F16X3, PG_PREC_F16X2)
_F16_PRECS = (PG_PREC_F16X3, PG_PREC_F16X2, PG_PREC_F16)
DEFAULT_BASE_OFFSET_MODE = 0


def _rows(L):
    return (L + 7) // 8 * 8


def layer_lengths(levels, T):
    Ld = [T]
    for lv in levels:
        Ld.append(lv.down.out_len(Ld[-1]))
        if Ld[-1] < 1:
            return None
    for i in range(len(levels) - 1, 0, -1):
        if levels[i].up.out_len(Ld[i + 1]) != Ld[i]:
            return None
    return Ld + [levels[0].up.out_len(Ld[1])]


def min_frames(levels, multiple=8, limit=1 << 16):
    for T in range(multiple, limit + 1, multiple):
        if layer_lengths(levels, T) is not None:
            return T
    raise ValueError("phasegen: no frame count up to %d fits this U-Net" % limit)


def clip_rows_table(levels, T_list):
    cols = []
    for T in T_list:
        L = layer_lengths(levels, int(T))
        if L is None:
            raise ValueError(f"phasegen: a clip of {T} frames does not fit this U-Net (minimum {min_frames(levels)}, "
                             "and the skip connections need T % 8 == 0)")
        cols.append(L)
    return [list(r) for r in zip(*cols)]


class ConvSpec:
    def __init__(self, kind, C_in, C_out, k, stride, pad):
        self.kind, self.C_in, self.C_out, self.k, self.stride, self.pad = kind, C_in, C_out, k, stride, pad

    def out_len(self, L):
        if self.kind == PG_CONV_TRANSPOSE:
            return (L - 1) * self.stride - 2 * self.pad + self.k
        return (L + 2 * self.pad - self.k) // self.stride + 1


class LevelSpec:

    def __init__(self, down, down_norm, up, up_norm=True):
        self.down, self.down_norm, self.up, self.up_norm = down, down_norm, up, up_norm


def tc_supported(levels):
    return all(l.down.C_in % 64 == 0 and l.down.C_out % 128 == 0 and l.up.C_in % 64 == 0 and l.up.C_out % 128 == 0
               for l in levels)


class _Operand:

    def __init__(self, B, L, ld, prec, device, range_flag=None):
        self.B, self.L, self.rows, self.ld = B, L, _rows(L), ld
        self.range_flag = range_flag if prec in _F16_PRECS else None
        if prec == PG_PREC_FP32_SIMT:
            self.dtype = PG_DT_F32
            self.hi = torch.zeros(B, self.rows, ld, device=device, dtype=torch.float32)
            self.lo = None
        elif prec == PG_PREC_F16:
            self.dtype = PG_DT_F16
            self.hi = torch.zeros(B, self.rows, ld, device=device, dtype=torch.float16)
            self.lo = None
        elif prec in _F16_PRECS:
            self.dtype = PG_DT_F16_SPLIT
            self.hi = torch.zeros(B, self.rows, ld, device=device, dtype=torch.float16)
            self.lo = torch.zeros_like(self.hi)
        else:
            self.dtype = PG_DT_BF16_SPLIT if prec == PG_PREC_BF16X3 else PG_DT_BF16
            self.hi = torch.zeros(B, self.rows, ld, device=device, dtype=torch.bfloat16)
            self.lo = torch.zeros_like(self.hi) if prec == PG_PREC_BF16X3 else None

    def dst(self, slope, ch_off=0):
        return ops.act_dst(self.hi, self.lo, self.rows * self.ld, self.ld, ch_off, self.dtype, slope, self.range_flag)

    def as_float(self):
        v = self.hi.float()
        if self.lo is not None:
            v = v + self.lo.float()
        return v[:, :self.L]


class UNetExecutor:
    def __init__(self, levels, B, T, device, precision="bf16x3", per_clip=False, out_channels=None,
                 taps_per_group=None, base_offset_mode=None, keep_raw=False, fast_layers=None, fuse=None,
                 use_running=False):
        self.levels, self.B, self.T, self.device = levels, B, T, torch.device(device)
        single_layers = ()
        if precision == "f16mix1":
            precision, single_layers = "f16mix", F16MIX1_SINGLE_LAYERS
        if precision == "f16mix":
            precision, fast_layers = "f16x3", (F16MIX_FAST_LAYERS if fast_layers is None else fast_layers)
        self.prec = PRECISIONS[precision] if isinstance(precision, str) else precision
        self.fast_layers = tuple(fast_layers or ()) if self.prec == PG_PREC_F16X3 else ()
        self.single_layers = tuple(single_layers) if self.prec == PG_PREC_F16X3 else ()
        if self.prec != PG_PREC_FP32_SIMT and not tc_supported(levels):
            raise RuntimeError("phasegen: tensor-core path needs C_in % 64 == 0 and C_out % 128 == 0 in every "
                               "layer; use precision='fp32_simt' for this channel count")
        self.per_clip, self.keep_raw, self.use_running = per_clip, keep_raw, bool(use_running)
        self.fuse = (self.prec != PG_PREC_FP32_SIMT and not keep_raw) if fuse is None else \
            bool(fuse and self.prec != PG_PREC_FP32_SIMT and not keep_raw)
        self.range_flag = torch.zeros(1, device=self.device, dtype=torch.int32)
        self.tpg = DEFAULT_TAPS_PER_GROUP if taps_per_group is None else taps_per_group
        self.bo = DEFAULT_BASE_OFFSET_MODE if base_offset_mode is None else base_offset_mode
        D = self.D = len(levels)
        dev, prec = self.device, self.prec
        self.Ld = [T]
        for lv in levels:
            self.Ld.append(lv.down.out_len(self.Ld[-1]))
            if self.Ld[-1] < 1:
                raise RuntimeError(f"phasegen: time axis too short for this U-Net (T={T})")
        for i in range(D - 1, 0, -1):
            got, want = levels[i].up.out_len(self.Ld[i + 1]), self.Ld[i]
            if got != want:
                raise RuntimeError(f"Sizes of tensors must match except in dimension 1. Expected size {want} "
                                   f"but got size {got} for the skip connection of level {i} (T={T}; "
                                   f"the reference U-Net needs T % 8 == 0 and T >= 24)")
        self.T_out = levels[0].up.out_len(self.Ld[1])
        self.C_final = levels[0].up.C_out if out_channels is None else out_channels
        G = B if per_clip else 1

        rf = self.range_flag
        self.x0 = _Operand(B, T, levels[0].down.C_in, prec, dev, rf)
        self.a, self.cat, self.z, self.g = [None] * D, [None] * D, [None] * D, [None] * D
        self.dn_desc, self.up_desc = [None] * D, [None] * D
        self.dn_mode, self.up_mode = [PG_EPI_RAW] * D, [PG_EPI_RAW] * D
        self.dn_stats, self.up_stats, self.dn_ss, self.up_ss = [None] * D, [None] * D, [None] * D, [None] * D
        self.dn_mv, self.up_mv = [None] * D, [None] * D
        for i, lv in enumerate(levels):
            Lz = self.Ld[i + 1]
            src = self.x0 if i == 0 else self.a[i - 1]
            if src.ld != lv.down.C_in:
                raise RuntimeError(f"phasegen: level {i} down conv expects {lv.down.C_in} channels, gets {src.ld}")
            self.a[i] = _Operand(B, Lz, lv.down.C_out, prec, dev, rf)
            if i < D - 1:
                cat_prec = PG_PREC_F16 if self.layer_prec("u", i) == PG_PREC_F16 else prec
                self.cat[i] = _Operand(B, Lz, lv.up.C_in, cat_prec, dev, rf)
                if lv.down.C_out + levels[i + 1].up.C_out != lv.up.C_in:
                    raise RuntimeError(f"phasegen: level {i}: concat width {lv.down.C_out}+{levels[i + 1].up.C_out} "
                                       f"!= up conv input {lv.up.C_in}")
            elif lv.up.C_in != lv.down.C_out:
                raise RuntimeError("phasegen: innermost up conv width mismatch")
            self.dn_desc[i] = ops.conv_desc(lv.down.kind, B, lv.down.C_in, lv.down.C_out, src.L, lv.down.k,
                                            lv.down.stride, lv.down.pad, src.rows, src.ld, self.layer_prec("d", i),
                                            taps_per_group=self.tpg, base_offset_mode=self.bo)
            up_src = self.a[i] if i == D - 1 else self.cat[i]
            c_out = self.C_final if i == 0 else lv.up.C_out
            self.up_desc[i] = ops.conv_desc(lv.up.kind, B, lv.up.C_in, c_out, up_src.L, lv.up.k, lv.up.stride,
                                            lv.up.pad, up_src.rows, up_src.ld, self.layer_prec("u", i),
                                            taps_per_group=self.tpg, base_offset_mode=self.bo)
            self.dn_mode[i] = self._pick_mode(self.dn_desc[i], lv.down_norm, last=False)
            self.up_mode[i] = self._pick_mode(self.up_desc[i], lv.up_norm, last=(i == 0))
            self.dn_stats[i], self.dn_ss[i], self.dn_mv[i] = self._stat_bufs(self.dn_desc[i], lv.down_norm and self.dn_mode[i] == PG_EPI_RAW, G)
            self.up_stats[i], self.up_ss[i], self.up_mv[i] = self._stat_bufs(self.up_desc[i], lv.up_norm and self.up_mode[i] == PG_EPI_RAW, G)
        sizes = [B * self.Ld[i + 1] * levels[i].down.C_out * (self.dn_mode[i] == PG_EPI_RAW) for i in range(D)] + \
                [B * (self.T_out if i == 0 else self.Ld[i]) * self.up_desc[i].C_out * (self.up_mode[i] == PG_EPI_RAW) for i in range(D)]
        if keep_raw:
            self.z = [torch.empty(s, device=dev, dtype=torch.float32) for s in sizes[:D]]
            self.g = [torch.empty(s, device=dev, dtype=torch.float32) for s in sizes[D:]]
        else:
            scratch = torch.empty(max(max(sizes), 1), device=dev, dtype=torch.float32)
            self.z = [scratch] * D
            self.g = [scratch] * D
        self._out = None
        self.weight_ready = None

    @property
    def out(self):
        if self._out is None:
            self._out = torch.empty(self.B, self.T_out, self.C_final, device=self.device, dtype=torch.float32)
        return self._out

    def _pick_mode(self, desc, has_norm, last):
        if not self.fuse or last:
            return PG_EPI_RAW
        if not has_norm:
            return PG_EPI_ACT
        if self.per_clip and not self.use_running and ops.conv_epilogue_supported(desc, PG_EPI_NORM_ACT):
            whole, split = ops.conv_plan(desc, whole_clip=1), ops.conv_plan(desc, whole_clip=0)
            if whole is not None and (whole["tiles"] >= whole["units"] or whole["tiles"] >= split["tiles"]) and \
                    whole["acc_stages"] >= split["acc_stages"]:
                return PG_EPI_NORM_ACT
        return PG_EPI_RAW

    def check_range(self):
        if int(self.range_flag.item()):
            self.range_flag.zero_()
            raise OverflowError("phasegen: an activation exceeded the fp16 range (|x| > 65504 or non-finite) in an fp16 "
                                "operand mode; results are invalid -- use precision='bf16x3' (bf16 planes, fp32 range)")

    def layer_prec(self, side, level):
        if self.prec == PG_PREC_F16X3 and f"{side}{level + 1}" in self.single_layers:
            return PG_PREC_F16
        if self.prec == PG_PREC_F16X3 and f"{side}{level + 1}" in self.fast_layers:
            return PG_PREC_F16X2
        return self.prec

    def _stat_bufs(self, desc, has_norm, G):
        if not has_norm:
            return None, None, None
        P = ops.conv_stat_parts(desc) if self.prec != PG_PREC_FP32_SIMT else 1
        stats = torch.empty(self.B, P, desc.C_out, 4, device=self.device, dtype=torch.float32)
        ss = torch.empty(G, desc.C_out, 2, device=self.device, dtype=torch.float32)
        mv = torch.empty(G, desc.C_out, 2, device=self.device, dtype=torch.float32)
        return stats, ss, mv

    def _pack_one(self, w, kind, slice_out=None, prec=None):
        prec = self.prec if prec is None else prec
        tc = prec != PG_PREC_FP32_SIMT
        if not tc:
            if slice_out is not None:
                w = w[:, :slice_out]
            return ops.pack_weight(w.contiguous(), kind, want_tc=False, want_simt=True)
        plane_dtype = torch.float16 if prec in _F16_PRECS else torch.bfloat16
        want_lo = prec in (PG_PREC_BF16X3, PG_PREC_F16X3)
        pv = ops.packed_view(w, kind)
        if pv is None:
            if slice_out is not None:
                w = w[:, :slice_out]
            return ops.pack_weight(w.contiguous(), kind, want_tc=True, want_simt=False, plane_dtype=plane_dtype, want_lo=want_lo)
        if slice_out is not None:
            pv = pv[:, :slice_out].contiguous()
        hi = torch.empty(pv.shape, device=pv.device, dtype=plane_dtype)
        lo = torch.empty_like(hi) if want_lo else None
        ops.cast_split(pv, hi, lo, self.range_flag if plane_dtype == torch.float16 else None)
        return hi, lo, None

    def pack_weights(self, down_w, up_w):
        self.wd, self.wu = [], []
        for i, lv in enumerate(self.levels):
            self.wd.append(self._pack_one(down_w[i], lv.down.kind, None, self.layer_prec("d", i)))
            sl = self.C_final if (i == 0 and self.C_final != lv.up.C_out) else None
            self.wu.append(self._pack_one(up_w[i], lv.up.kind, sl, self.layer_prec("u", i)))

    def _conv(self, desc, src, w, y, stats, rows=None):
        if self.weight_ready is not None:
            self.weight_ready(w)
        if rows is not None:
            ops.conv_tc(desc, src.hi, src.lo, w[0], w[1], y, stats, out_rows=rows)
            return
        if self.prec == PG_PREC_FP32_SIMT:
            ops.conv_simt(desc, src.hi, w[2], y)
            if stats is not None:
                ops.channel_stats(y, desc.B, desc.L_out, desc.C_out, desc.out_rows, desc.out_ld, stats)
        else:
            ops.conv_tc(desc, src.hi, src.lo, w[0], w[1], y, stats)

    def _finalize(self, desc, stats, ss, mv, norm, running):
        gamma, beta, eps = norm
        if self.use_running:
            if running is None:
                raise RuntimeError("phasegen: executor built with use_running=True needs the running statistics")
            ops.bn_from_running(running[0], running[1], gamma, beta, eps, ss, mv)
        else:
            ops.bn_finalize(stats, desc.B, stats.shape[1], desc.C_out, self.per_clip, gamma, beta, eps, ss, mv)

    def _layer(self, mode, desc, src, w, y, stats, ss, mv, norm, running, dst0, dst1=None, rows=None):
        if mode != PG_EPI_RAW:
            if self.weight_ready is not None:
                self.weight_ready(w)
            gamma, beta, eps = norm if norm is not None else (None, None, BN_EPS_DEFAULT)
            ops.conv_tc(desc, src.hi, src.lo, w[0], w[1], None, None,
                        ops.conv_epilogue(mode, dst0, dst1, gamma, beta, eps), out_rows=rows)
            return
        self._conv(desc, src, w, y, stats, rows)
        if stats is not None:
            self._finalize(desc, stats, ss, mv, norm, running)
        ops.bn_act(y, desc.B, desc.L_out, desc.C_out, desc.out_rows, desc.out_ld,
                   ss if stats is not None else None, self.per_clip, dst0, dst1, clip_rows=rows)

    def load_input_cf(self, x):
        B, Cn, T = x.shape
        ops.transpose(x, dst=self.x0.hi if self.x0.dtype == PG_DT_F32 else None,
                      dst_hi=None if self.x0.dtype == PG_DT_F32 else self.x0.hi, dst_lo=self.x0.lo,
                      dst_batch_stride=self.x0.rows * self.x0.ld, dst_ld=self.x0.ld, range_flag=self.x0.range_flag)

    def load_input_cl(self, x_cl):
        B, T, Cn = x_cl.shape
        ops.bn_act(x_cl, B, T, Cn, T, Cn, None, False, self.x0.dst(1.0))

    def run(self, dn_norm, up_norm, defer_last=False, dn_running=None, up_running=None, clip_rows=None):
        D, lv = self.D, self.levels
        if clip_rows is not None:
            if self.prec == PG_PREC_FP32_SIMT or not self.per_clip:
                raise ValueError("phasegen: ragged batches need per-clip statistics and a tensor-core precision")
            if tuple(clip_rows.shape) != (D + 2, self.B) or clip_rows.dtype != torch.int32:
                raise ValueError(f"phasegen: clip_rows must be int32 [{D + 2}, {self.B}]")
        rows = (lambda j: clip_rows[j]) if clip_rows is not None else (lambda j: None)
        run_of = lambda lst, i: lst[i] if lst is not None else None
        for i in range(D):
            src = self.x0 if i == 0 else self.a[i - 1]
            norm = dn_norm[i] if lv[i].down_norm else None
            dsts = (self.a[i].dst(0.2), self.cat[i].dst(0.0, 0)) if i < D - 1 else (self.a[i].dst(0.0), None)
            self._layer(self.dn_mode[i], self.dn_desc[i], src, self.wd[i], self.z[i], self.dn_stats[i], self.dn_ss[i],
                        self.dn_mv[i], norm, run_of(dn_running, i), *dsts, rows=rows(i + 1))
        for i in range(D - 1, 0, -1):
            src = self.a[i] if i == D - 1 else self.cat[i]
            norm = up_norm[i] if lv[i].up_norm else None
            self._layer(self.up_mode[i], self.up_desc[i], src, self.wu[i], self.g[i], self.up_stats[i], self.up_ss[i],
                        self.up_mv[i], norm, run_of(up_running, i), self.cat[i - 1].dst(0.0, lv[i - 1].down.C_out), rows=rows(i))
        src = self.a[0] if D == 1 else self.cat[0]
        desc, y, stats = self.up_desc[0], self.g[0], self.up_stats[0]
        self._conv(desc, src, self.wu[0], y, stats, rows(D + 1))
        norm = up_norm[0] if lv[0].up_norm else None
        if norm is not None and self.C_final != lv[0].up.C_out:
            norm = (norm[0][:self.C_final] if norm[0] is not None else None,
                    norm[1][:self.C_final] if norm[1] is not None else None, norm[2])
        running = run_of(up_running, 0)
        if running is not None and self.C_final != lv[0].up.C_out:
            running = (running[0][:self.C_final], running[1][:self.C_final])
        if stats is not None:
            self._finalize(desc, stats, self.up_ss[0], self.up_mv[0], norm, running)
        if defer_last and stats is not None:
            return y[:self.B * self.T_out * self.C_final].view(self.B, self.T_out, self.C_final), self.up_ss[0]
        ops.bn_act(y, desc.B, desc.L_out, desc.C_out, desc.out_rows, desc.out_ld, self.up_ss[0] if stats is not None else None,
                   self.per_clip, ops.act_dst(self.out, None, self.T_out * self.C_final, self.C_final, 0, PG_DT_F32, 1.0),
                   clip_rows=rows(D + 1))
        return self.out
```

Measured before the change: 45960.

## Add staged epilogue with eight warps and register rebalancing for single-stage accumulators

Doubles the kernel to 384 threads with eight epilogue warps, using setmaxnreg to shift registers from the producer/MMA warps to the epilogue. When the accumulator is single-staged and a tile holds two units, each epilogue warp-group loads its whole TMEM slice into registers up front and releases the accumulator before computing stats and stores. This lets the next tile's MMA overlap with the epilogue work. It also lets the fused norm+act epilogue be chosen in more cases. The cost is heavy register pressure (176-float arrays per thread) and a different shared-memory budget, which may reduce A-stage slots.

```diff
diff --git a/unet-phasegen_b200/csrc/api.cu b/unet-phasegen_b200/csrc/api.cu
--- a/unet-phasegen_b200/csrc/api.cu
+++ b/unet-phasegen_b200/csrc/api.cu
@@ -64,5 +64,6 @@
                        p.n_chunks, p.n_cotiles, p.OS, p.IS, p.n_taps[0], p.n_taps[1], p.n_groups[0], p.n_groups[1]};
     for (int i = 0; i < 16; ++i) out[i] = v[i];
     if (n_out >= 17) out[16] = p.whole_clip;
+    if (n_out >= 18) out[17] = p.epi_staged;
     return PG_OK;
 }
diff --git a/unet-phasegen_b200/csrc/conv_plan.h b/unet-phasegen_b200/csrc/conv_plan.h
--- a/unet-phasegen_b200/csrc/conv_plan.h
+++ b/unet-phasegen_b200/csrc/conv_plan.h
@@ -8,6 +8,7 @@
 namespace pg {
 
 constexpr int kMaxTaps = 32;
+constexpr int kStageCols = 176;
 
 struct ConvTap { int8_t w_idx; int8_t shift; int8_t parity; int8_t pad_; int32_t d; };
 struct ConvGroup { int32_t row0; int8_t parity; int8_t n_taps; int8_t first_tap; int8_t pad_; };
@@ -25,6 +26,7 @@
     int merged;
     int clip_group;
     int whole_clip;
+    int epi_staged;
     int out_rows, out_ld;
     int n_groups[2], n_taps[2];
     ConvGroup groups[2][kMaxTaps];
@@ -177,6 +179,11 @@
         if (cols > 512) { set_error("conv plan: tile needs %d accumulator columns (> 512)", cols); return PG_ERR_UNSUPPORTED; }
         p->acc_stages = cols <= 256 ? 2 : 1;
     }
+    {
+        const int units = p->merged ? 0 : p->nb * (p->whole_clip ? p->OS * p->n_ntiles : 1);
+        const char* e = getenv("PG_TC_EPI_DRAIN");
+        p->epi_staged = (p->acc_stages == 1 && units == 2 && p->n_tile <= kStageCols && !(e && atoi(e) == 1)) ? 1 : 0;
+    }
     p->clip_group = d->B;
     return PG_OK;
 }
diff --git a/unet-phasegen_b200/csrc/conv_tc.cu b/unet-phasegen_b200/csrc/conv_tc.cu
--- a/unet-phasegen_b200/csrc/conv_tc.cu
+++ b/unet-phasegen_b200/csrc/conv_tc.cu
@@ -20,11 +20,22 @@
     const int* clip_rows;
 };
 
-constexpr int kThreads = 192;
+constexpr int kThreads = 384;
+constexpr int kEpiWarps = 8;
+constexpr int kRegsLaunch = (65536 / kThreads) & ~7;
+constexpr int kRegsIssue = 40, kRegsEpi = 232;
+static_assert(128 * kRegsIssue + 256 * kRegsEpi <= kThreads * kRegsLaunch, "setmaxnreg budgets exceed the launch allocation");
+constexpr int kEpiSmemStaged = kEpiWarps * (2048 + 256), kEpiSmemDrain = 4 * 2048;
 constexpr int kATileBytes = 128 * 128;
 constexpr int kMaxASlots = 8;
 
 struct TileCoord { int co_tile, phase, b0, nt; };
+
+template <int N>
+__device__ __forceinline__ void shift16(float (&v)[N]) {
+#pragma unroll
+    for (int i = 0; i + 16 < N; ++i) v[i] = v[i + 16];
+}
 
 __device__ __forceinline__ int n_bundles(const ConvPlan& p) { return (p.B + p.nb - 1) / p.nb; }
 __device__ __forceinline__ int n_co_slabs(const ConvPlan& p) { return p.pair ? p.n_cotiles / 2 : p.n_cotiles; }
@@ -44,6 +55,20 @@
     c.b0 = (g * G + r2 / NTx) * p.nb; c.nt = r2 % NTx;
     return c;
 }
+
+#define PG_CONV_ROLE_VARS                                                                                               \
+    const int n_tiles = total_tiles(pl);                                                                                \
+    const bool w_lo = prm.n_terms == 3, x_lo = prm.n_terms >= 2;                                                        \
+    const int rank = PAIR ? (int)cluster_ctarank() : 0;                               \
+    const int tile0 = PAIR ? (int)(blockIdx.x >> 1) : (int)blockIdx.x;                                                  \
+    const int tile_step = PAIR ? (int)(gridDim.x >> 1) : (int)gridDim.x;                                                \
+    const int half_n = pl.n_tile >> 1;                             \
+    const int nb_grp = pl.nb / pl.mgroups;                         \
+    const int nb_cta = (PAIR && pl.merged) ? nb_grp >> 1 : nb_grp;    \
+    const int t_phases = pl.whole_clip ? pl.OS : 1;                \
+    const int t_nts = pl.whole_clip ? pl.n_ntiles : 1;                                                                  \
+    const int n_sub = pl.merged ? pl.mgroups : t_nts;                              \
+    (void)n_tiles; (void)w_lo; (void)x_lo; (void)rank; (void)half_n; (void)nb_grp; (void)nb_cta; (void)n_sub;
 
 template <bool PAIR, bool RAGGED>
 __global__ void __launch_bounds__(kThreads, 1)
@@ -68,19 +93,18 @@
     uint64_t* accEmpty = accFull + 2;
     uint32_t* tmem_slot = reinterpret_cast<uint32_t*>(accEmpty + 2);
     uint32_t* epi_tiles = reinterpret_cast<uint32_t*>(reinterpret_cast<uint8_t*>(bars) + 256);
+    float* epi_xch = reinterpret_cast<float*>(epi_tiles + kEpiWarps * 512);
 
     const int warp = __shfl_sync(0xffffffffu, (int)(threadIdx.x >> 5), 0), lane = threadIdx.x & 31;
-    const int n_tiles = total_tiles(pl);
-    const bool w_lo = prm.n_terms == 3, x_lo = prm.n_terms >= 2;
 
     if (warp == 0 && lane == 0) {
         tma_prefetch_desc(&map_w_hi); tma_prefetch_desc(&map_x_hi);
-        if (w_lo) tma_prefetch_desc(&map_w_lo);
-        if (x_lo) tma_prefetch_desc(&map_x_lo);
+        if (prm.n_terms == 3) tma_prefetch_desc(&map_w_lo);
+        if (prm.n_terms >= 2) tma_prefetch_desc(&map_x_lo);
         for (int i = 0; i < nA; ++i) { mbar_init(fullA + i, 1); mbar_init(emptyA + i, 1); }
         for (int i = 0; i < 2; ++i) {
             mbar_init(fullB + i, 1); mbar_init(emptyB + i, 1);
-            mbar_init(accFull + i, 1); mbar_init(accEmpty + i, PAIR ? 8 : 4);
+            mbar_init(accFull + i, 1); mbar_init(accEmpty + i, PAIR ? 2 * kEpiWarps : kEpiWarps);
         }
         fence_barrier_init();
     }
@@ -89,17 +113,10 @@
     if (PAIR) cluster_sync_all(); else __syncthreads();
     tc_fence_after();
     const uint32_t tmem_base = __shfl_sync(0xffffffffu, *tmem_slot, 0);
-    const int rank = PAIR ? (int)cluster_ctarank() : 0;
-    const int tile0 = PAIR ? (int)(blockIdx.x >> 1) : (int)blockIdx.x;
-    const int tile_step = PAIR ? (int)(gridDim.x >> 1) : (int)gridDim.x;
-    const int half_n = pl.n_tile >> 1;
-    const int nb_grp = pl.nb / pl.mgroups;
-    const int nb_cta = (PAIR && pl.merged) ? nb_grp >> 1 : nb_grp;
-    const int t_phases = pl.whole_clip ? pl.OS : 1;
-    const int t_nts = pl.whole_clip ? pl.n_ntiles : 1;
-    const int n_sub = pl.merged ? pl.mgroups : t_nts;
-
-    if (warp == 0) {
+    if (warp < 4) {
+      setmaxnreg_dec<kRegsIssue>();
+      PG_CONV_ROLE_VARS
+      if (warp == 0) {
         {
             uint32_t b_it = 0;
             int a_slot = 0; uint32_t a_ph = 0;
@@ -118,7 +135,7 @@
                         const ConvGroup grp = pl.groups[ph][g];
                         {
                             const int s = b_it & 1; const uint32_t bph = (b_it >> 1) & 1;
-                            mbar_wait(emptyB + s, bph ^ 1);
+                            mbar_wait<false>(emptyB + s, bph ^ 1);
                             uint8_t* dst = b_base + (size_t)s * b_planes * bPlane;
                             if (elect_one()) {
                                 if (PAIR) { if (rank == 0) mbar_expect_tx(fullB + s, 2 * b_bytes); }
@@ -142,7 +159,7 @@
                         for (int j = 0; j < grp.n_taps; ++j) {
                             const int w_idx = pl.taps[ph][grp.first_tap + j].w_idx;
                             const int s = a_slot; const uint32_t aph = a_ph;
-                            mbar_wait(emptyA + s, aph ^ 1);
+                            mbar_wait<false>(emptyA + s, aph ^ 1);
                             uint8_t* dst = a_base + (size_t)s * a_planes * kATileBytes;
                             if (elect_one()) {
                                 if (!PAIR) mbar_expect_tx(fullA + s, a_bytes);
@@ -169,7 +186,7 @@
                 }
             }
         }
-    } else if (warp == 1) {
+      } else if (warp == 1) {
         if (rank == 0) {
             uint32_t b_it = 0, t_it = 0;
             int a_slot = 0; uint32_t a_ph = 0;
@@ -191,7 +208,7 @@
                 TileCoord tc = decode_tile(pl, tile);
                 const int acc = pl.acc_stages == 2 ? (t_it & 1) : 0;
                 const uint32_t acc_ph = pl.acc_stages == 2 ? ((t_it >> 1) & 1) : (t_it & 1);
-                mbar_wait_sleep(accEmpty + acc, acc_ph ^ 1, 200);
+                mbar_wait_sleep<false>(accEmpty + acc, acc_ph ^ 1, 200);
                 tc_fence_after();
                 const uint32_t d_tmem = tmem_base + acc * 256;
                 const uint32_t strip_bytes = (uint32_t)pl.strip_rows * 128u;
@@ -203,14 +220,14 @@
                     for (int g = 0; g < ng; ++g) {
                         const ConvGroup grp = pl.groups[ph][g];
                         const int bs = b_it & 1; const uint32_t bph = (b_it >> 1) & 1;
-                        mbar_wait(fullB + bs, bph);
+                        mbar_wait<false>(fullB + bs, bph);
                         tc_fence_after();
                         const uint32_t b_hi = smem_u32(b_base + (size_t)bs * b_planes * bPlane);
                         const uint32_t b_lo = b_hi + bPlane;
                         for (int j = 0; j < grp.n_taps; ++j) {
                             const ConvTap tp = pl.taps[ph][grp.first_tap + j];
                             const int as = a_slot; const uint32_t aph = a_ph;
-                            mbar_wait(fullA + as, aph);
+                            mbar_wait<false>(fullA + as, aph);
                             tc_fence_after();
                             const uint32_t a_hi = smem_u32(a_base + (size_t)as * a_planes * kATileBytes);
                             const uint32_t a_lo = a_hi + kATileBytes;
@@ -252,9 +269,14 @@
                 commit(accFull + acc);
             }
         }
+      }
     } else {
-        const int q = warp & 3;
-        uint32_t* tile = epi_tiles + q * 512;
+        setmaxnreg_inc<kRegsEpi>();
+        PG_CONV_ROLE_VARS
+        const int e = warp - 4, q = warp & 3, h = e >> 2;
+        uint32_t* tile = epi_tiles + e * 512;
+        float* xch = epi_xch + e * 64;
+        const float* xch_peer = epi_xch + (e ^ 4) * 64;
         uint32_t t_it = 0;
         const int n_parts = t_phases * t_nts;
         const int col_pitch = pl.merged ? pl.strip_rows : pl.n_tile * n_parts;
@@ -308,8 +330,13 @@
             if (PAIR) tc.co_tile = tc.co_tile * 2 + rank;
             const int acc = pl.acc_stages == 2 ? (t_it & 1) : 0;
             const uint32_t acc_ph = pl.acc_stages == 2 ? ((t_it >> 1) & 1) : (t_it & 1);
-            mbar_wait_sleep(accFull + acc, acc_ph, 1000);
+            mbar_wait_sleep<false>(accFull + acc, acc_ph, 1000);
             tc_fence_after();
+            auto release = [&]() {
+                tc_fence_before();
+                __syncwarp();
+                if (lane == 0) { if (PAIR) mbar_arrive_leader(accEmpty + acc); else mbar_arrive(accEmpty + acc); }
+            };
             const int co_base = tc.co_tile * 128 + q * 32;
             const int co = co_base + lane;
             auto part_geom = [&](int p, int L, int& phase, int& m0, int& n_valid) {
@@ -318,107 +345,186 @@
                 const int l_phase = (L - phase + pl.OS - 1) / pl.OS;
                 n_valid = l_phase - m0; if (n_valid > pl.n_tile) n_valid = pl.n_tile; if (n_valid < 0) n_valid = 0;
             };
-            for (int c = 0; c < pl.nb; ++c) {
+            auto raw_chunk = [&](const float* v, float mean, float& m2, int b, int phase, int m0, int c0, int n_valid) {
+#pragma unroll
+                for (int i = 0; i < 16; ++i) if (c0 + i < n_valid) { const float d = v[i] - mean; m2 += d * d; }
+                const size_t off0 = ((size_t)b * pl.out_rows + (size_t)(m0 + c0) * pl.OS + phase) * pl.out_ld + co_base;
+                store_f32(prm.y, off0, (size_t)pl.OS * pl.out_ld, v, n_valid - c0);
+            };
+            auto raw_stats = [&](int b, int phase, int m0, int n_valid, float mean, float m2) {
+                if (prm.stats) {
+                    const int P = pl.OS * pl.n_ntiles;
+                    const int pi = phase * pl.n_ntiles + m0 / pl.n_tile;
+                    prm.stats[((size_t)b * P + pi) * pl.C_out + co] = make_float4((float)n_valid, mean, m2, 0.f);
+                }
+            };
+            auto norm_coeffs = [&](int b, int n_tot, float mean, float m2, float& sc, float& sh, bool record) {
+                const float var = n_tot > 0 ? m2 / (float)n_tot : 0.f;
+                sc = (prm.gamma ? __ldg(prm.gamma + co) : 1.f) * rsqrtf(var + prm.eps);
+                sh = (prm.beta ? __ldg(prm.beta + co) : 0.f) - mean * sc;
+                if (record && prm.ss_out) prm.ss_out[(size_t)b * pl.C_out + co] = make_float2(sc, sh);
+            };
+            auto act_chunk = [&](const float* vin, float sc, float sh, int b, int phase, int m0, int c0, int n_valid, int n_own) {
+                float v[16];
+#pragma unroll
+                for (int i = 0; i < 16; ++i) v[i] = fmaf(vin[i], sc, sh);
+                if (RAGGED) {
+#pragma unroll
+                    for (int i = 0; i < 16; ++i) if (c0 + i >= n_own) v[i] = 0.f;
+                }
+                const size_t row0 = (size_t)(m0 + c0) * pl.OS + phase;
+#pragma unroll
+                for (int k = 0; k < 2; ++k) {
+                    const ActDst& d = k ? prm.dst1 : prm.dst0;
+                    if (!d.dtype) continue;
+                    const size_t off0 = (size_t)b * d.batch_stride + row0 * d.ld + d.ch_off + co_base;
+                    if (d.dtype == PG_DT_F32) {
+                        float a[16];
+#pragma unroll
+                        for (int i = 0; i < 16; ++i) a[i] = leaky(v[i], d.slope);
+                        store_f32(static_cast<float*>(d.hi), off0, (size_t)pl.OS * d.ld, a, n_valid - c0);
+                    } else {
+                        store_split(d, off0, (size_t)pl.OS * d.ld, v, n_valid - c0);
+                    }
+                }
+            };
+            if (pl.epi_staged) {
+                const int c = n_parts == 2 ? 0 : h, p = n_parts == 2 ? h : 0;
                 const int b = tc.b0 + c;
-                if (b >= pl.B) break;
-                const int L_b = RAGGED ? min(__ldg(prm.clip_rows + b), pl.L_out) : pl.L_out;
-                const uint32_t tclip = tmem_base + acc * 256 + c * col_pitch + ((uint32_t)(q * 32) << 16);
-                if (prm.epi_mode == PG_EPI_RAW) {
-                    for (int p = 0; p < n_parts; ++p) {
-                        int phase, m0, n_valid;
-                        part_geom(p, L_b, phase, m0, n_valid);
-                        const uint32_t taddr = tclip + p * pl.n_tile;
+                uint32_t r[kStageCols];
+                const uint32_t taddr = tmem_base + c * col_pitch + p * pl.n_tile + ((uint32_t)(q * 32) << 16);
+#pragma unroll
+                for (int j = 0; j < kStageCols / 32; ++j) tmem_ld32_nowait(taddr + 32 * j, r + 32 * j);
+                if (kStageCols % 32) tmem_ld16_nowait(taddr + kStageCols / 32 * 32, r + kStageCols / 32 * 32);
+                tmem_wait_ld<kStageCols>(r);
+                release();
+                float v[kStageCols];
+#pragma unroll
+                for (int i = 0; i < kStageCols; ++i) v[i] = __uint_as_float(r[i]);
+                if (b < pl.B) {
+                    const int L_b = RAGGED ? min(__ldg(prm.clip_rows + b), pl.L_out) : pl.L_out;
+                    int phase, m0, n_valid;
+                    part_geom(p, L_b, phase, m0, n_valid);
+                    auto valid_sum = [&]() {
                         float sum = 0.f;
-                        for (int c0 = 0; c0 < n_valid; c0 += 16) {
-                            float v[16];
-                            tmem_ld16(taddr + c0, v);
-#pragma unroll
-                            for (int i = 0; i < 16; ++i) if (c0 + i < n_valid) sum += v[i];
-                        }
+#pragma unroll
+                        for (int i = 0; i < kStageCols; ++i) if (i < n_valid) sum += v[i];
+                        return sum;
+                    };
+                    if (prm.epi_mode == PG_EPI_RAW) {
+                        const float sum = valid_sum();
                         const float mean = n_valid > 0 ? sum / (float)n_valid : 0.f;
                         float m2 = 0.f;
-                        const size_t row_pitch = (size_t)pl.OS * pl.out_ld;
+#pragma unroll 1
                         for (int c0 = 0; c0 < n_valid; c0 += 16) {
-                            float v[16];
-                            tmem_ld16(taddr + c0, v);
-#pragma unroll
-                            for (int i = 0; i < 16; ++i) if (c0 + i < n_valid) { const float d = v[i] - mean; m2 += d * d; }
-                            const size_t off0 = ((size_t)b * pl.out_rows + (size_t)(m0 + c0) * pl.OS + phase) * pl.out_ld + co_base;
-                            store_f32(prm.y, off0, row_pitch, v, n_valid - c0);
-                        }
-                        if (prm.stats) {
-                            const int P = pl.OS * pl.n_ntiles;
-                            const int pi = phase * pl.n_ntiles + m0 / pl.n_tile;
-                            prm.stats[((size_t)b * P + pi) * pl.C_out + co] = make_float4((float)n_valid, mean, m2, 0.f);
+                            raw_chunk(v, mean, m2, b, phase, m0, c0, n_valid);
+                            shift16(v);
+                        }
+                        raw_stats(b, phase, m0, n_valid, mean, m2);
+                    } else {
+                        float sc = 1.f, sh = 0.f;
+                        if (prm.epi_mode == PG_EPI_NORM_ACT) {
+                            float sum = valid_sum();
+                            int n_tot = n_valid;
+                            if (n_parts == 2) {
+                                int ph_, m0_, nv_;
+                                part_geom(p ^ 1, L_b, ph_, m0_, nv_);
+                                n_tot += nv_;
+                                xch[lane] = sum;
+                                named_bar_sync(1 + q, 64);
+                                sum = h == 0 ? sum + xch_peer[lane] : xch_peer[lane] + sum;
+                            }
+                            const float mean = n_tot > 0 ? sum / (float)n_tot : 0.f;
+                            float m2 = 0.f;
+#pragma unroll
+                            for (int i = 0; i < kStageCols; ++i) if (i < n_valid) { const float d = v[i] - mean; m2 += d * d; }
+                            if (n_parts == 2) {
+                                xch[32 + lane] = m2;
+                                named_bar_sync(1 + q, 64);
+                                m2 = h == 0 ? m2 + xch_peer[32 + lane] : xch_peer[32 + lane] + m2;
+                            }
+                            norm_coeffs(b, n_tot, mean, m2, sc, sh, n_parts == 1 || h == 0);
+                        }
+                        int n_out, n_own = 0;
+                        part_geom(p, pl.L_out, phase, m0, n_out);
+                        if (RAGGED) n_own = n_valid;
+#pragma unroll 1
+                        for (int c0 = 0; c0 < n_out; c0 += 16) {
+                            act_chunk(v, sc, sh, b, phase, m0, c0, n_out, n_own);
+                            shift16(v);
                         }
                     }
-                } else {
-                    float sc = 1.f, sh = 0.f;
-                    if (prm.epi_mode == PG_EPI_NORM_ACT) {
-                        float sum = 0.f; int n_tot = 0;
+                }
+            } else {
+                for (int c = 0; c < (h == 0 ? pl.nb : 0); ++c) {
+                    const int b = tc.b0 + c;
+                    if (b >= pl.B) break;
+                    const int L_b = RAGGED ? min(__ldg(prm.clip_rows + b), pl.L_out) : pl.L_out;
+                    const uint32_t tclip = tmem_base + acc * 256 + c * col_pitch + ((uint32_t)(q * 32) << 16);
+                    if (prm.epi_mode == PG_EPI_RAW) {
                         for (int p = 0; p < n_parts; ++p) {
                             int phase, m0, n_valid;
                             part_geom(p, L_b, phase, m0, n_valid);
-                            n_tot += n_valid;
+                            const uint32_t taddr = tclip + p * pl.n_tile;
+                            float sum = 0.f;
+                            for (int c0 = 0; c0 < n_valid; c0 += 16) {
+                                float v[16];
+                                tmem_ld16(taddr + c0, v);
+#pragma unroll
+                                for (int i = 0; i < 16; ++i) if (c0 + i < n_valid) sum += v[i];
+                            }
+                            const float mean = n_valid > 0 ? sum / (float)n_valid : 0.f;
+                            float m2 = 0.f;
+                            for (int c0 = 0; c0 < n_valid; c0 += 16) {
+                                float v[16];
+                                tmem_ld16(taddr + c0, v);
+                                raw_chunk(v, mean, m2, b, phase, m0, c0, n_valid);
+                            }
+                            raw_stats(b, phase, m0, n_valid, mean, m2);
+                        }
+                    } else {
+                        float sc = 1.f, sh = 0.f;
+                        if (prm.epi_mode == PG_EPI_NORM_ACT) {
+                            float sum = 0.f; int n_tot = 0;
+                            for (int p = 0; p < n_parts; ++p) {
+                                int phase, m0, n_valid;
+                                part_geom(p, L_b, phase, m0, n_valid);
+                                n_tot += n_valid;
+                                for (int c0 = 0; c0 < n_valid; c0 += 16) {
+                                    float v[16];
+                                    tmem_ld16(tclip + p * pl.n_tile + c0, v);
+#pragma unroll
+                                    for (int i = 0; i < 16; ++i) if (c0 + i < n_valid) sum += v[i];
+                                }
+                            }
+                            const float mean = n_tot > 0 ? sum / (float)n_tot : 0.f;
+                            float m2 = 0.f;
+                            for (int p = 0; p < n_parts; ++p) {
+                                int phase, m0, n_valid;
+                                part_geom(p, L_b, phase, m0, n_valid);
+                                for (int c0 = 0; c0 < n_valid; c0 += 16) {
+                                    float v[16];
+                                    tmem_ld16(tclip + p * pl.n_tile + c0, v);
+#pragma unroll
+                                    for (int i = 0; i < 16; ++i) if (c0 + i < n_valid) { const float d = v[i] - mean; m2 += d * d; }
+                                }
+                            }
+                            norm_coeffs(b, n_tot, mean, m2, sc, sh, true);
+                        }
+                        for (int p = 0; p < n_parts; ++p) {
+                            int phase, m0, n_valid, n_own = 0;
+                            part_geom(p, pl.L_out, phase, m0, n_valid);
+                            if (RAGGED) { int ph_, m0_; part_geom(p, L_b, ph_, m0_, n_own); }
                             for (int c0 = 0; c0 < n_valid; c0 += 16) {
                                 float v[16];
                                 tmem_ld16(tclip + p * pl.n_tile + c0, v);
-#pragma unroll
-                                for (int i = 0; i < 16; ++i) if (c0 + i < n_valid) sum += v[i];
-                            }
-                        }
-                        const float mean = n_tot > 0 ? sum / (float)n_tot : 0.f;
-                        float m2 = 0.f;
-                        for (int p = 0; p < n_parts; ++p) {
-                            int phase, m0, n_valid;
-                            part_geom(p, L_b, phase, m0, n_valid);
-                            for (int c0 = 0; c0 < n_valid; c0 += 16) {
-                                float v[16];
-                                tmem_ld16(tclip + p * pl.n_tile + c0, v);
-#pragma unroll
-                                for (int i = 0; i < 16; ++i) if (c0 + i < n_valid) { const float d = v[i] - mean; m2 += d * d; }
-                            }
-                        }
-                        const float var = n_tot > 0 ? m2 / (float)n_tot : 0.f;
-                        sc = (prm.gamma ? __ldg(prm.gamma + co) : 1.f) * rsqrtf(var + prm.eps);
-                        sh = (prm.beta ? __ldg(prm.beta + co) : 0.f) - mean * sc;
-                        if (prm.ss_out) prm.ss_out[(size_t)b * pl.C_out + co] = make_float2(sc, sh);
+                                act_chunk(v, sc, sh, b, phase, m0, c0, n_valid, n_own);
+                            }
+                        }
                     }
-                    for (int p = 0; p < n_parts; ++p) {
-                        int phase, m0, n_valid, n_own = 0;
-                        part_geom(p, pl.L_out, phase, m0, n_valid);
-                        if (RAGGED) { int ph_, m0_; part_geom(p, L_b, ph_, m0_, n_own); }
-                        for (int c0 = 0; c0 < n_valid; c0 += 16) {
-                            float v[16];
-                            tmem_ld16(tclip + p * pl.n_tile + c0, v);
-#pragma unroll
-                            for (int i = 0; i < 16; ++i) v[i] = fmaf(v[i], sc, sh);
-                            if (RAGGED) {
-#pragma unroll
-                                for (int i = 0; i < 16; ++i) if (c0 + i >= n_own) v[i] = 0.f;
-                            }
-                            const size_t row0 = (size_t)(m0 + c0) * pl.OS + phase;
-#pragma unroll
-                            for (int k = 0; k < 2; ++k) {
-                                const ActDst& d = k ? prm.dst1 : prm.dst0;
-                                if (!d.dtype) continue;
-                                const size_t off0 = (size_t)b * d.batch_stride + row0 * d.ld + d.ch_off + co_base;
-                                if (d.dtype == PG_DT_F32) {
-                                    float a[16];
-#pragma unroll
-                                    for (int i = 0; i < 16; ++i) a[i] = leaky(v[i], d.slope);
-                                    store_f32(static_cast<float*>(d.hi), off0, (size_t)pl.OS * d.ld, a, n_valid - c0);
-                                } else {
-                                    store_split(d, off0, (size_t)pl.OS * d.ld, v, n_valid - c0);
-                                }
-                            }
-                        }
-                    }
-                }
+                }
+                release();
             }
-            tc_fence_before();
-            __syncwarp();
-            if (lane == 0) { if (PAIR) mbar_arrive_leader(accEmpty + acc); else mbar_arrive(accEmpty + acc); }
         }
         if (bad_range) {
             if (prm.dst0.range_flag) atomicOr(prm.dst0.range_flag, 1);
@@ -537,7 +643,8 @@
     const int nb_cta = (pl.pair && pl.merged) ? nb_grp / 2 : nb_grp;
     prm.b_slot_bytes = (pl.merged ? pl.mgroups : (pl.whole_clip ? pl.n_ntiles : 1)) * nb_cta * pl.strip_rows * 128;
     const int a_planes = n_terms == 3 ? 2 : 1, b_planes = n_terms >= 2 ? 2 : 1;
-    const int fixed = 2 * b_planes * prm.b_slot_bytes + 1024  + 256  + 8192  +
+    const int fixed = 2 * b_planes * prm.b_slot_bytes + 1024  + 256  +
+                      (pl.epi_staged ? kEpiSmemStaged : kEpiSmemDrain) +
                       (pl.merged ? 2048 : 0);
     int nA = (g_max_smem - fixed) / (a_planes * kATileBytes);
     if (nA > kMaxASlots) nA = kMaxASlots;
@@ -570,6 +677,16 @@
         static size_t configured_dev[kMaxDevices][4] = {};
         const int variant = 2 * pair + ragged;
         size_t* configured = configured_dev[current_device_slot()];
+        if (!configured[variant]) {
+            cudaFuncAttributes fa;
+            cudaError_t e = cudaFuncGetAttributes(&fa, kernel);
+            if (e != cudaSuccess) { set_error("conv_tc: cudaFuncGetAttributes failed: %s", cudaGetErrorString(e)); return PG_ERR_CUDA; }
+            if (fa.numRegs * kThreads < 128 * kRegsIssue + 256 * kRegsEpi) {
+                set_error("conv_tc: kernel built with %d registers per thread; its setmaxnreg budgets (%d / %d) need %d", fa.numRegs,
+                          kRegsIssue, kRegsEpi, kRegsLaunch);
+                return PG_ERR_UNSUPPORTED;
+            }
+        }
         if (smem_bytes > configured[variant]) {
             cudaError_t e = cudaFuncSetAttribute(kernel, cudaFuncAttributeMaxDynamicSharedMemorySize, (int)smem_bytes);
             if (e != cudaSuccess) { set_error("conv_tc: cannot opt in to %zu bytes of shared memory: %s", smem_bytes, cudaGetErrorString(e)); return PG_ERR_CUDA; }
diff --git a/unet-phasegen_b200/csrc/tc_ptx.cuh b/unet-phasegen_b200/csrc/tc_ptx.cuh
--- a/unet-phasegen_b200/csrc/tc_ptx.cuh
+++ b/unet-phasegen_b200/csrc/tc_ptx.cuh
@@ -28,24 +28,26 @@
         : "=r"(ok) : "r"(smem_u32(bar)), "r"(parity) : "memory");
     return ok != 0;
 }
+template <bool kReport = true>
 __device__ __forceinline__ void mbar_wait(uint64_t* bar, uint32_t parity) {
     if (mbar_try_wait(bar, parity)) return;
     const long long t0 = clock64();
     for (uint32_t spins = 1; !mbar_try_wait(bar, parity); ++spins) {
         if ((spins & 1023u) == 0 && clock64() - t0 > 4000000000ll) {
-            printf("phasegen conv_tc: mbarrier timeout (block %d thread %d bar %u parity %u)\n",
+            if (kReport) printf("phasegen conv_tc: mbarrier timeout (block %d thread %d bar %u parity %u)\n",
                    (int)blockIdx.x, (int)threadIdx.x, smem_u32(bar), parity);
             __trap();
         }
     }
 }
+template <bool kReport = true>
 __device__ __forceinline__ void mbar_wait_sleep(uint64_t* bar, uint32_t parity, unsigned ns) {
     if (mbar_try_wait(bar, parity)) return;
     const long long t0 = clock64();
     for (uint32_t spins = 1; !mbar_try_wait(bar, parity); ++spins) {
         __nanosleep(ns);
         if ((spins & 255u) == 0 && clock64() - t0 > 4000000000ll) {
-            printf("phasegen conv_tc: mbarrier timeout (block %d thread %d bar %u parity %u)\n",
+            if (kReport) printf("phasegen conv_tc: mbarrier timeout (block %d thread %d bar %u parity %u)\n",
                    (int)blockIdx.x, (int)threadIdx.x, smem_u32(bar), parity);
             __trap();
         }
@@ -102,6 +104,35 @@
     asm volatile("tcgen05.wait::ld.sync.aligned;" ::: "memory");
 #pragma unroll
     for (int i = 0; i < 16; ++i) v[i] = __uint_as_float(r[i]);
+}
+__device__ __forceinline__ void tmem_ld16_nowait(uint32_t taddr, uint32_t* r) {
+    asm volatile(
+        "tcgen05.ld.sync.aligned.32x32b.x16.b32 {%0,%1,%2,%3,%4,%5,%6,%7,%8,%9,%10,%11,%12,%13,%14,%15}, [%16];"
+        : "=r"(r[0]), "=r"(r[1]), "=r"(r[2]), "=r"(r[3]), "=r"(r[4]), "=r"(r[5]), "=r"(r[6]), "=r"(r[7]),
+          "=r"(r[8]), "=r"(r[9]), "=r"(r[10]), "=r"(r[11]), "=r"(r[12]), "=r"(r[13]), "=r"(r[14]), "=r"(r[15])
+        : "r"(taddr));
+}
+__device__ __forceinline__ void tmem_ld32_nowait(uint32_t taddr, uint32_t* r) {
+    asm volatile(
+        "tcgen05.ld.sync.aligned.32x32b.x32.b32 {%0,%1,%2,%3,%4,%5,%6,%7,%8,%9,%10,%11,%12,%13,%14,%15,"
+        "%16,%17,%18,%19,%20,%21,%22,%23,%24,%25,%26,%27,%28,%29,%30,%31}, [%32];"
+        : "=r"(r[0]), "=r"(r[1]), "=r"(r[2]), "=r"(r[3]), "=r"(r[4]), "=r"(r[5]), "=r"(r[6]), "=r"(r[7]),
+          "=r"(r[8]), "=r"(r[9]), "=r"(r[10]), "=r"(r[11]), "=r"(r[12]), "=r"(r[13]), "=r"(r[14]), "=r"(r[15]),
+          "=r"(r[16]), "=r"(r[17]), "=r"(r[18]), "=r"(r[19]), "=r"(r[20]), "=r"(r[21]), "=r"(r[22]), "=r"(r[23]),
+          "=r"(r[24]), "=r"(r[25]), "=r"(r[26]), "=r"(r[27]), "=r"(r[28]), "=r"(r[29]), "=r"(r[30]), "=r"(r[31])
+        : "r"(taddr));
+}
+template <int N>
+__device__ __forceinline__ void tmem_wait_ld(uint32_t* r) {
+    asm volatile("tcgen05.wait::ld.sync.aligned;" ::: "memory");
+#pragma unroll
+    for (int i = 0; i < N; ++i) asm volatile("" : "+r"(r[i]));
+}
+
+template <int R> __device__ __forceinline__ void setmaxnreg_dec() { asm volatile("setmaxnreg.dec.sync.aligned.u32 %0;" ::"n"(R)); }
+template <int R> __device__ __forceinline__ void setmaxnreg_inc() { asm volatile("setmaxnreg.inc.sync.aligned.u32 %0;" ::"n"(R)); }
+__device__ __forceinline__ void named_bar_sync(int id, int count) {
+    asm volatile("bar.sync %0, %1;" ::"r"(id), "r"(count) : "memory");
 }
 
 constexpr uint32_t kPeerBitMask = 0xFEFFFFFFu;
diff --git a/unet-phasegen_b200/phasegen/ops.py b/unet-phasegen_b200/phasegen/ops.py
--- a/unet-phasegen_b200/phasegen/ops.py
+++ b/unet-phasegen_b200/phasegen/ops.py
@@ -217,15 +217,15 @@
 
 
 _PLAN_KEYS = ("n_tile", "n_ntiles", "nb", "strip_rows", "pair", "merged", "mgroups", "acc_stages", "n_chunks", "n_cotiles",
-              "OS", "IS", "taps0", "taps1", "groups0", "groups1", "whole_clip")
+              "OS", "IS", "taps0", "taps1", "groups0", "groups1", "whole_clip", "epi_staged")
 
 
 def conv_plan(desc, whole_clip=None):
     d = ConvDesc.from_buffer_copy(desc)
     if whole_clip is not None:
         d.tc_whole_clip = int(whole_clip)
-    out = (C.c_int * 17)()
-    if _lib.load().pg_conv_tc_plan(C.byref(d), out, 17) != 0:
+    out = (C.c_int * 18)()
+    if _lib.load().pg_conv_tc_plan(C.byref(d), out, 18) != 0:
         return None
     pl = dict(zip(_PLAN_KEYS, out))
     slabs = pl["n_cotiles"] // 2 if pl["pair"] else pl["n_cotiles"]
diff --git a/unet-phasegen_b200/phasegen/unet.py b/unet-phasegen_b200/phasegen/unet.py
--- a/unet-phasegen_b200/phasegen/unet.py
+++ b/unet-phasegen_b200/phasegen/unet.py
@@ -199,7 +199,7 @@
         if self.per_clip and not self.use_running and ops.conv_epilogue_supported(desc, PG_EPI_NORM_ACT):
             whole, split = ops.conv_plan(desc, whole_clip=1), ops.conv_plan(desc, whole_clip=0)
             if whole is not None and (whole["tiles"] >= whole["units"] or whole["tiles"] >= split["tiles"]) and \
-                    whole["acc_stages"] >= split["acc_stages"]:
+                    ((whole["epi_staged"] and whole["OS"] == 1) or whole["acc_stages"] >= split["acc_stages"]):
                 return PG_EPI_NORM_ACT
         return PG_EPI_RAW
 
```

Measured after the change: 47340 (median of 6 runs). 1.03x the previous value.
